# yang-song/score_sde_pytorch

Hardware: AMD Instinct MI355X
Metric: pc_sampler_images_per_sec (higher is better)
Workload: dtype f32 via 3-way bf16 split, fp32 accumulate (the 1x1 / NIN / Linear GEMMs and the attention forward as exact-fp32 products on the BF16 matrix pipe, fp32 softmax; 3x3 convolutions and the attention backward on the fp32-MFMA kernels); 1 GPU; configs/ve/cifar10_ncsnpp_continuous PC sampler (reverse_diffusion+langevin), batch 256/GPU, N=1000, 32x32; 1 step = 1 PC iteration = 2 U-Net evaluations; batch_per_gpu=256, sde_steps=1000, state_finite=True, matrix_mode=bf16x6, parallelism=replicas x1 (no collectives)

## Files before the change

### include/ssde.h

```cpp
#ifndef SSDE_H_
#define SSDE_H_

#include <stddef.h>
#include <stdint.h>

#ifdef __cplusplus
extern "C" {
#endif

#define SSDE_ABI_VERSION 12

enum {
  SSDE_PRO_NONE = 0,
  SSDE_PRO_GN = 1,
  SSDE_PRO_GN_SILU = 2,
  SSDE_PRO_SILU = 3
};

typedef struct ssde_src {
  const float* p0;
  const float* p1;
  int32_t c0, c1;
  int32_t pro_mode;
  int32_t gn_groups;
  const float* gn_mean;
  const float* gn_rstd;
  const float* gn_gamma;
  const float* gn_beta;
  uint32_t drop_thresh;
  float drop_scale;
  const uint32_t* drop_seed;
  uint32_t drop_salt;
  int32_t _pad;
} ssde_src;

typedef struct ssde_conv_args {
  ssde_src main;
  ssde_src aux;
  const float* w_main;
  const float* w_aux;
  int32_t n, h_in, w_in;
  int32_t h_out, w_out, c_out;
  int32_t ksize;
  int32_t stride;
  int32_t pad;
  int32_t tile;
  const float* bias;
  const float* chan_add;
  int32_t chan_add_ld;
  int32_t resid_post;
  const float* resid;
  float out_scale;
  uint32_t flags;
  float* dst;
  float* gn_part;
  float* wino_v;
  const float* gn_in_part0;
  const float* gn_in_part1;
  int32_t gn_in_slices0, gn_in_slices1;
  float gn_in_eps;
  int32_t pad_end;
  float* wino_ws;
  int64_t wino_ws_floats;
} ssde_conv_args;

enum { SSDE_CONVF_V_GIVEN = 1u,
       SSDE_CONVF_BF16X6 = 2u,
       SSDE_CONVF_NO_KSPLIT = 4u,
       SSDE_CONVF_BKC8 = 8u,
       SSDE_CONVF_GEMM_PIPE = 16u,
       SSDE_CONVF_NO_GEMM_PIPE = 32u,
       SSDE_CONVF_X6_BM64 = 64u,
       SSDE_CONVF_X6_PF2 = 128u,
       SSDE_CONVF_NO_SMALL_COUT = 256u,
       SSDE_CONVF_X6_WIDE = 512u,
       SSDE_CONVF_X6_NO_WIDE = 1024u,
       SSDE_CONVF_KSPLIT2 = 2048u,
       SSDE_CONVF_KSPLIT4 = 4096u };
enum { SSDE_TILE_AUTO = 0, SSDE_TILE_256x64 = 1, SSDE_TILE_128x64 = 2, SSDE_TILE_64x64 = 3, SSDE_TILE_256x32 = 4,
       SSDE_TILE_WINOGRAD = 5,
       SSDE_TILE_WINOGRAD4 = 6,
       SSDE_TILE_WINOGRAD4R = 9,
       SSDE_TILE_WINOGRAD4P = 10 };

typedef struct ssde_gn_stats_args {
  const float* p0; const float* p1; int32_t c0, c1;
  int32_t n, hw, groups; float eps;
  float* mean; float* rstd;
  float* scratch;
  int32_t slices; int32_t _pad0;
} ssde_gn_stats_args;

typedef struct ssde_gn_finalize_args {
  const float* part0; const float* part1;
  int32_t c0, c1, slices0, slices1;
  int32_t n, groups; float eps; int32_t _pad0;
  float* mean; float* rstd;
} ssde_gn_finalize_args;

typedef struct ssde_upfirdn_args {
  ssde_src src;
  int32_t n, h_in, w_in, c;
  int32_t h_out, w_out;
  int32_t up, down, pad0, pad1;
  int32_t kh, kw;
  float k[16];
  float* dst;
  int32_t accumulate;
  int32_t _pad0;
  float* dst2;
} ssde_upfirdn_args;

typedef struct ssde_attn_args {
  const float* qkv; float* dst;
  int32_t n, l, c; float scale;
  uint32_t flags;
  int32_t _pad0;
} ssde_attn_args;
enum { SSDE_ATTNF_BF16X6 = 1u };

typedef struct ssde_embed_args {
  const float* cond;
  const float* w;
  float* dst;
  int32_t n, dim, kind, _pad0;
} ssde_embed_args;

typedef struct ssde_to_nhwc_args {
  const float* src; float* dst; int32_t n, c, h, w, c_pad; float a, b;
  int32_t mode;
  const float* v;
} ssde_to_nhwc_args;
typedef struct ssde_to_nchw_args {
  const float* src; float* dst; int32_t n, c, h, w, c_src;
  int32_t mode;
  const float* v;
  float alpha;
  int32_t accumulate;
} ssde_to_nchw_args;

typedef struct ssde_bias_act_args {
  const float* src; const float* bias; float* dst;
  int64_t numel; int32_t channels; int32_t inner;
  int32_t act;
  float alpha, scale;
  int32_t grad;
  const float* ref;
} ssde_bias_act_args;

typedef struct ssde_sumsq_args {
  const float* a; const float* b; float* out_a; float* out_b; int32_t n, per;
} ssde_sumsq_args;
typedef struct ssde_randn_args {
  float* dst; int64_t numel; uint64_t seed; const int32_t* step_ptr; int32_t stream_id; int32_t _pad0;
  const uint64_t* seed_ptr;
} ssde_randn_args;
typedef struct ssde_langevin_args {
  float* x; float* x_mean; const float* grad; const float* noise;
  const float* grad_sumsq; const float* noise_sumsq;
  const float* alpha_tab; const int32_t* step_ptr;
  int32_t n, per; float snr; int32_t _pad0;
} ssde_langevin_args;
typedef struct ssde_predictor_args {
  float* x; float* x_mean; const float* score; const float* noise;
  const float* coef; const int32_t* step_ptr;
  int64_t numel;
} ssde_predictor_args;
typedef struct ssde_sample_update_args {
  const float* x; const float* y; const float* z; const float* a; const float* b; const float* c;
  float* x_mean; float* x_out; int32_t n; int32_t per;
} ssde_sample_update_args;
typedef struct ssde_fill_args {
  float* dst; const float* tab; const int32_t* step_ptr; int32_t n; int32_t _pad0;
} ssde_fill_args;
typedef struct ssde_step_inc_args { int32_t* step_ptr; int32_t delta; int32_t _pad0; } ssde_step_inc_args;
typedef struct ssde_project_args {
  float* x; float* x_mean; const float* data; const float* mask; const float* noise;
  const float* coef; const int32_t* step_ptr;
  int32_t n, c, hw;
  int32_t use_matrix;
  float M[9], invM[9];
} ssde_project_args;



typedef struct ssde_wgrad_args {
  ssde_src src;
  const float* g;
  int32_t g_ld, g_off;
  int32_t n, h_in, w_in, h_out, w_out;
  int32_t c_out;
  int32_t ksize;
  int32_t stride, pad;
  int32_t cin_store;
  int32_t transpose_out;
  int32_t splits;
  float scale;
  uint32_t flags;
  float* dw;
  float* scratch;
  int64_t scratch_floats;
  const float* v_pre;
// ... 277 lines not shown
```

### score_sde_pytorch_amd/_lib.py

```python
import ctypes as C
import os

_HERE = os.path.dirname(os.path.abspath(__file__))
LIB_PATH = os.environ.get("SSDE_LIB_PATH") or os.path.join(_HERE, "libssde_hip.so")
ABI_VERSION = 12

PRO_NONE, PRO_GN, PRO_GN_SILU, PRO_SILU = 0, 1, 2, 3
TILE_AUTO, TILE_256x64, TILE_128x64, TILE_64x64, TILE_256x32, TILE_WINOGRAD, TILE_WINOGRAD4 = 0, 1, 2, 3, 4, 5, 6
TILE_WINOGRAD4R = 9
TILE_WINOGRAD4P = 10
TILES_WINOGRAD4 = (TILE_WINOGRAD4, TILE_WINOGRAD4R, TILE_WINOGRAD4P)
CONVF_V_GIVEN, CONVF_BF16X6, CONVF_NO_KSPLIT, CONVF_BKC8, CONVF_GEMM_PIPE, CONVF_NO_GEMM_PIPE, CONVF_X6_BM64, CONVF_X6_PF2, \
    CONVF_NO_SMALL_COUT, CONVF_X6_WIDE, CONVF_X6_NO_WIDE, CONVF_KSPLIT2, CONVF_KSPLIT4 = 1, 2, 4, 8, 16, 32, 64, 128, 256, 512, 1024, 2048, 4096
WGRADF_DIRECT, WGRADF_F2, WGRADF_F4_FORCE, WGRADF_NO_STREAMK, WGRADF_NO_XCD_ORDER, WGRADF_1X1_CHUNKED, WGRADF_XVEC1 = 1, 2, 4, 8, 16, 32, 64
GNBWDF_THREE_KERNELS, GNBWDF_DEFER_PARAMS = 1, 2
(OP_CONV, OP_GN_STATS, OP_UPFIRDN, OP_ATTN, OP_EMBED, OP_TO_NHWC, OP_TO_NCHW, OP_BIAS_ACT, OP_SUMSQ,
 OP_RANDN, OP_LANGEVIN, OP_PREDICTOR, OP_FILL, OP_STEP_INC, OP_WGRAD, OP_COLSUM, OP_GN_BWD_REDUCE, OP_PROLOGUE_BWD,
 OP_ATTN_BWD, OP_PERTURB, OP_DSM_LOSS, OP_SUMSQ_FLAT, OP_ADAM, OP_MEMSET, OP_AXPY, OP_PACK, OP_PROJECT,
 OP_GN_FINALIZE, OP_PF_DRIFT, OP_HUTCH_DIV, OP_COLSUM_FINISH, OP_GN_BWD_FINISH) = range(1, 33)
FINISH_JOBS = 16
COLSUMF_DEFER = 1
PACK_CONV3, PACK_WINO3, PACK_MATRIX, PACK_VECTOR, PACK_WINO4, PACK_WINO4R, PACK_WINO4P = 1, 2, 3, 4, 5, 6, 7

_fp = C.c_void_p


class Src(C.Structure):
    _fields_ = [("p0", _fp), ("p1", _fp), ("c0", C.c_int32), ("c1", C.c_int32),
                ("pro_mode", C.c_int32), ("gn_groups", C.c_int32),
                ("gn_mean", _fp), ("gn_rstd", _fp), ("gn_gamma", _fp), ("gn_beta", _fp),
                ("drop_thresh", C.c_uint32), ("drop_scale", C.c_float), ("drop_seed", _fp),
                ("drop_salt", C.c_uint32), ("_pad", C.c_int32)]


class ConvArgs(C.Structure):
    _fields_ = [("main", Src), ("aux", Src), ("w_main", _fp), ("w_aux", _fp),
                ("n", C.c_int32), ("h_in", C.c_int32), ("w_in", C.c_int32),
                ("h_out", C.c_int32), ("w_out", C.c_int32), ("c_out", C.c_int32),
                ("ksize", C.c_int32), ("stride", C.c_int32), ("pad", C.c_int32), ("tile", C.c_int32),
                ("bias", _fp), ("chan_add", _fp), ("chan_add_ld", C.c_int32), ("resid_post", C.c_int32),
                ("resid", _fp), ("out_scale", C.c_float), ("flags", C.c_uint32), ("dst", _fp), ("gn_part", _fp), ("wino_v", _fp),
                ("gn_in_part0", _fp), ("gn_in_part1", _fp), ("gn_in_slices0", C.c_int32), ("gn_in_slices1", C.c_int32),
                ("gn_in_eps", C.c_float), ("pad_end", C.c_int32), ("wino_ws", _fp), ("wino_ws_floats", C.c_int64)]


class GnStatsArgs(C.Structure):
    _fields_ = [("p0", _fp), ("p1", _fp), ("c0", C.c_int32), ("c1", C.c_int32),
                ("n", C.c_int32), ("hw", C.c_int32), ("groups", C.c_int32), ("eps", C.c_float),
                ("mean", _fp), ("rstd", _fp), ("scratch", _fp), ("slices", C.c_int32), ("_pad0", C.c_int32)]


class RkCombineArgs(C.Structure):
    _fields_ = [("y", _fp), ("k", _fp), ("n", C.c_int64), ("terms", C.c_int32), ("_pad0", C.c_int32), ("coef", C.c_double * 7),
                ("dst", _fp), ("dst32", _fp), ("n32", C.c_int64)]


class RkErrorArgs(C.Structure):
    _fields_ = [("y", _fp), ("y_new", _fp), ("k", _fp), ("n", C.c_int64), ("coef", C.c_double * 7), ("atol", C.c_double),
                ("rtol", C.c_double), ("partial", _fp), ("partial_len", C.c_int32), ("_pad0", C.c_int32), ("out", _fp)]


class PfDriftArgs(C.Structure):
    _fields_ = [("x", _fp), ("score", _fp), ("dst", _fp), ("numel", C.c_int64), ("a", C.c_float), ("g2", C.c_float), ("dyn", _fp)]


class OdeDyn(C.Structure):
    _fields_ = [("label", C.c_float), ("std", C.c_float), ("a", C.c_float), ("g2", C.c_float), ("dst", _fp)]


class HutchDivArgs(C.Structure):
    _fields_ = [("gx", _fp), ("eps", _fp), ("dst", _fp), ("dst_off", C.c_int64), ("n", C.c_int32), ("per", C.c_int32),
                ("a", C.c_float), ("g2", C.c_float), ("dyn", _fp)]


class GnFinalizeArgs(C.Structure):
    _fields_ = [("part0", _fp), ("part1", _fp), ("c0", C.c_int32), ("c1", C.c_int32), ("slices0", C.c_int32), ("slices1", C.c_int32),
                ("n", C.c_int32), ("groups", C.c_int32), ("eps", C.c_float), ("_pad0", C.c_int32), ("mean", _fp), ("rstd", _fp)]


class UpfirdnArgs(C.Structure):
    _fields_ = [("src", Src), ("n", C.c_int32), ("h_in", C.c_int32), ("w_in", C.c_int32), ("c", C.c_int32),
                ("h_out", C.c_int32), ("w_out", C.c_int32),
                ("up", C.c_int32), ("down", C.c_int32), ("pad0", C.c_int32), ("pad1", C.c_int32),
                ("kh", C.c_int32), ("kw", C.c_int32), ("k", C.c_float * 16), ("dst", _fp),
                ("accumulate", C.c_int32), ("_pad0", C.c_int32), ("dst2", _fp)]


class AttnArgs(C.Structure):
    _fields_ = [("qkv", _fp), ("dst", _fp), ("n", C.c_int32), ("l", C.c_int32), ("c", C.c_int32), ("scale", C.c_float),
                ("flags", C.c_uint32), ("_pad0", C.c_int32)]


class EmbedArgs(C.Structure):
    _fields_ = [("cond", _fp), ("w", _fp), ("dst", _fp), ("n", C.c_int32), ("dim", C.c_int32),
                ("kind", C.c_int32), ("_pad0", C.c_int32)]


class ToNhwcArgs(C.Structure):
    _fields_ = [("src", _fp), ("dst", _fp), ("n", C.c_int32), ("c", C.c_int32), ("h", C.c_int32), ("w", C.c_int32),
                ("c_pad", C.c_int32), ("a", C.c_float), ("b", C.c_float), ("mode", C.c_int32), ("v", _fp)]


class ToNchwArgs(C.Structure):
    _fields_ = [("src", _fp), ("dst", _fp), ("n", C.c_int32), ("c", C.c_int32), ("h", C.c_int32), ("w", C.c_int32),
                ("c_src", C.c_int32), ("mode", C.c_int32), ("v", _fp), ("alpha", C.c_float), ("accumulate", C.c_int32)]


class BiasActArgs(C.Structure):
    _fields_ = [("src", _fp), ("bias", _fp), ("dst", _fp), ("numel", C.c_int64), ("channels", C.c_int32),
                ("inner", C.c_int32), ("act", C.c_int32), ("alpha", C.c_float), ("scale", C.c_float), ("grad", C.c_int32),
                ("ref", _fp)]


class SumsqArgs(C.Structure):
    _fields_ = [("a", _fp), ("b", _fp), ("out_a", _fp), ("out_b", _fp), ("n", C.c_int32), ("per", C.c_int32)]


class RandnArgs(C.Structure):
    _fields_ = [("dst", _fp), ("numel", C.c_int64), ("seed", C.c_uint64), ("step_ptr", _fp),
                ("stream_id", C.c_int32), ("_pad0", C.c_int32), ("seed_ptr", _fp)]


class LangevinArgs(C.Structure):
    _fields_ = [("x", _fp), ("x_mean", _fp), ("grad", _fp), ("noise", _fp), ("grad_sumsq", _fp), ("noise_sumsq", _fp),
                ("alpha_tab", _fp), ("step_ptr", _fp), ("n", C.c_int32), ("per", C.c_int32), ("snr", C.c_float),
                ("_pad0", C.c_int32)]


class PredictorArgs(C.Structure):
    _fields_ = [("x", _fp), ("x_mean", _fp), ("score", _fp), ("noise", _fp), ("coef", _fp), ("step_ptr", _fp),
                ("numel", C.c_int64)]


class SampleUpdateArgs(C.Structure):
    _fields_ = [("x", _fp), ("y", _fp), ("z", _fp), ("a", _fp), ("b", _fp), ("c", _fp), ("x_mean", _fp), ("x_out", _fp),
                ("n", C.c_int32), ("per", C.c_int32)]


class FillArgs(C.Structure):
    _fields_ = [("dst", _fp), ("tab", _fp), ("step_ptr", _fp), ("n", C.c_int32), ("_pad0", C.c_int32)]


class StepIncArgs(C.Structure):
    _fields_ = [("step_ptr", _fp), ("delta", C.c_int32), ("_pad0", C.c_int32)]


class ProjectArgs(C.Structure):
    _fields_ = [("x", _fp), ("x_mean", _fp), ("data", _fp), ("mask", _fp), ("noise", _fp), ("coef", _fp), ("step_ptr", _fp),
                ("n", C.c_int32), ("c", C.c_int32), ("hw", C.c_int32), ("use_matrix", C.c_int32),
                ("M", C.c_float * 9), ("invM", C.c_float * 9)]


class WgradArgs(C.Structure):
    _fields_ = [("src", Src), ("g", _fp), ("g_ld", C.c_int32), ("g_off", C.c_int32),
                ("n", C.c_int32), ("h_in", C.c_int32), ("w_in", C.c_int32), ("h_out", C.c_int32), ("w_out", C.c_int32),
                ("c_out", C.c_int32), ("ksize", C.c_int32), ("stride", C.c_int32), ("pad", C.c_int32),
                ("cin_store", C.c_int32), ("transpose_out", C.c_int32), ("splits", C.c_int32), ("scale", C.c_float),
                ("flags", C.c_uint32), ("dw", _fp), ("scratch", _fp), ("scratch_floats", C.c_int64), ("v_pre", _fp),
                ("pad_end", C.c_int32), ("_pad0", C.c_int32)]


class ColsumArgs(C.Structure):
    _fields_ = [("g", _fp), ("g_ld", C.c_int32), ("g_off", C.c_int32), ("n", C.c_int32), ("hw", C.c_int32),
                ("c", C.c_int32), ("scale", C.c_float), ("per_sample", _fp), ("ps_ld", C.c_int32), ("ps_off", C.c_int32),
                ("total", _fp), ("total2", _fp), ("scratch", _fp), ("flags", C.c_uint32), ("_pad0", C.c_int32)]


class ColsumJob(C.Structure):
    _fields_ = [("part", _fp), ("per_sample", _fp), ("total", _fp), ("total2", _fp), ("n", C.c_int32), ("slices", C.c_int32),
                ("c", C.c_int32), ("ps_ld", C.c_int32), ("ps_off", C.c_int32), ("_pad0", C.c_int32)]


class ColsumFinishArgs(C.Structure):
# ... 47 lines not shown
    _fields_ = [("dst", _fp), ("bytes", C.c_int64), ("value", C.c_int32), ("_pad0", C.c_int32)]


class AxpyArgs(C.Structure):
    _fields_ = [("x", _fp), ("gate", _fp), ("dst", _fp), ("numel", C.c_int64), ("alpha", C.c_float), ("acc", C.c_int32)]


class PackDesc(C.Structure):
    _fields_ = [("src", _fp), ("src2", _fp), ("dst", _fp), ("kind", C.c_int32), ("cout", C.c_int32), ("cin", C.c_int32),
                ("cout_l", C.c_int32), ("cin_l", C.c_int32), ("flags", C.c_int32), ("r_off", C.c_int32), ("c_off", C.c_int32),
                ("n", C.c_int64)]


class PackArgs(C.Structure):
    _fields_ = [("table", _fp), ("count", C.c_int32), ("kind", C.c_int32), ("max_n", C.c_int64)]


class _OpUnion(C.Union):
    _fields_ = [("conv", ConvArgs), ("gn", GnStatsArgs), ("fir", UpfirdnArgs), ("attn", AttnArgs),
                ("embed", EmbedArgs), ("to_nhwc", ToNhwcArgs), ("to_nchw", ToNchwArgs), ("bias_act", BiasActArgs),
                ("sumsq", SumsqArgs), ("randn", RandnArgs), ("langevin", LangevinArgs), ("predictor", PredictorArgs),
                ("fill", FillArgs), ("step_inc", StepIncArgs),
                ("wgrad", WgradArgs), ("colsum", ColsumArgs), ("gn_bwd", GnBwdReduceArgs), ("pro_bwd", PrologueBwdArgs),
                ("attn_bwd", AttnBwdArgs), ("perturb", PerturbArgs), ("dsm_loss", DsmLossArgs),
                ("sumsq_flat", SumsqFlatArgs), ("adam", AdamArgs), ("memset", MemsetArgs), ("axpy", AxpyArgs),
                ("pack", PackArgs), ("project", ProjectArgs), ("gn_fin", GnFinalizeArgs),
                ("pf_drift", PfDriftArgs), ("hutch_div", HutchDivArgs), ("colsum_fin", ColsumFinishArgs), ("gn_bwd_fin", GnBwdFinishArgs)]


class Op(C.Structure):
    _fields_ = [("kind", C.c_int32), ("flops_class", C.c_int32), ("u", _OpUnion)]


_UNION_FIELD = {OP_CONV: "conv", OP_GN_STATS: "gn", OP_UPFIRDN: "fir", OP_ATTN: "attn", OP_EMBED: "embed",
                OP_TO_NHWC: "to_nhwc", OP_TO_NCHW: "to_nchw", OP_BIAS_ACT: "bias_act", OP_SUMSQ: "sumsq",
                OP_RANDN: "randn", OP_LANGEVIN: "langevin", OP_PREDICTOR: "predictor", OP_FILL: "fill",
                OP_STEP_INC: "step_inc", OP_WGRAD: "wgrad", OP_COLSUM: "colsum", OP_GN_BWD_REDUCE: "gn_bwd",
                OP_PROLOGUE_BWD: "pro_bwd", OP_ATTN_BWD: "attn_bwd", OP_PERTURB: "perturb", OP_DSM_LOSS: "dsm_loss",
                OP_SUMSQ_FLAT: "sumsq_flat", OP_ADAM: "adam", OP_MEMSET: "memset", OP_AXPY: "axpy", OP_PACK: "pack", OP_PROJECT: "project",
                OP_GN_FINALIZE: "gn_fin", OP_PF_DRIFT: "pf_drift", OP_HUTCH_DIV: "hutch_div", OP_COLSUM_FINISH: "colsum_fin",
                OP_GN_BWD_FINISH: "gn_bwd_fin"}

EXPORTS = ["ssde_conv2d", "ssde_groupnorm_stats", "ssde_upfirdn2d", "ssde_attention", "ssde_embed", "ssde_to_nhwc",
           "ssde_to_nchw", "ssde_fused_bias_act", "ssde_sumsq", "ssde_randn", "ssde_langevin_update",
           "ssde_predictor_update", "ssde_fill_from_table", "ssde_step_inc", "ssde_program_run",
           "ssde_program_run_timed", "ssde_graph_capture", "ssde_graph_launch", "ssde_graph_destroy",
           "ssde_abi_version", "ssde_sizeof_op", "ssde_last_error", "ssde_conv_lds_bytes",
           "ssde_conv_wgrad", "ssde_colsum", "ssde_gn_bwd_reduce", "ssde_prologue_bwd", "ssde_attention_bwd",
           "ssde_perturb", "ssde_dsm_loss", "ssde_sumsq_flat", "ssde_adam_clip_ema", "ssde_memset", "ssde_axpy",
           "ssde_wgrad_scratch_floats", "ssde_wgrad_wants_winograd4", "ssde_pack_weights", "ssde_project_update", "ssde_gn_finalize", "ssde_conv_gn_slices", "ssde_conv_ws_floats", "ssde_rk_combine", "ssde_rk_error_norm", "ssde_pf_drift", "ssde_hutch_div", "ssde_sample_update", "ssde_mfma_probe", "ssde_colsum_finish", "ssde_gn_bwd_finish", "ssde_gn_bwd_scratch_rows",
           "ssde_plan_load", "ssde_plan_load_file", "ssde_plan_destroy", "ssde_plan_info", "ssde_plan_param",
           "ssde_plan_refresh_weights", "ssde_unet_forward", "ssde_pc_reset", "ssde_pc_run", "ssde_pc_state",
           "ssde_train_step", "ssde_train_forward", "ssde_unet_backward", "ssde_plan_copy_io"]

_lib = None


def conv_route_flags(env=None):
    e = os.environ if env is None else env
    f = 0
    if e.get("SSDE_MATRIX", "").startswith("b"):
        f |= CONVF_BF16X6
    if e.get("SSDE_CONV_KSPLIT", "1") == "0":
        f |= CONVF_NO_KSPLIT
    if e.get("SSDE_CONV_BKC64", "") == "8":
        f |= CONVF_BKC8
    if e.get("SSDE_GEMM_PIPE", "") == "0":
        f |= CONVF_NO_GEMM_PIPE
    if e.get("SSDE_GEMM_PIPE", "") == "2":
        f |= CONVF_GEMM_PIPE
    if e.get("SSDE_X6_BM", "") == "64":
        f |= CONVF_X6_BM64
    if e.get("SSDE_X6_PF", "") == "2":
        f |= CONVF_X6_PF2
    if e.get("SSDE_CONV_SMALL", "1") == "0":
        f |= CONVF_NO_SMALL_COUT
    if e.get("SSDE_X6_WIDE", "") == "1":
        f |= CONVF_X6_WIDE
    if e.get("SSDE_X6_WIDE", "") == "0":
        f |= CONVF_X6_NO_WIDE
    return f


ATTNF_BF16X6 = 1


def attn_route_flags(env=None):
    e = os.environ if env is None else env
    return ATTNF_BF16X6 if e.get("SSDE_MATRIX", "").startswith("b") and e.get("SSDE_ATTN_X6", "1") != "0" else 0


def wgrad_route_flags(env=None):
    e = os.environ if env is None else env
    f = {"0": WGRADF_DIRECT, "2": WGRADF_F2, "44": WGRADF_F4_FORCE}.get(e.get("SSDE_WGRAD_WINOGRAD", ""), 0)
    if e.get("SSDE_WGRAD4_STREAMK", "1") == "0":
        f |= WGRADF_NO_STREAMK
    if e.get("SSDE_WGRAD4_XCD", "1") == "0":
        f |= WGRADF_NO_XCD_ORDER
    if e.get("SSDE_WGRAD_1X1_PIPELINED", "1") == "0":
        f |= WGRADF_1X1_CHUNKED
    if e.get("SSDE_WGRAD4_XVEC", "2") == "1":
        f |= WGRADF_XVEC1
    return f


def gn_bwd_route_flags(env=None):
    e = os.environ if env is None else env
    return GNBWDF_THREE_KERNELS if e.get("SSDE_GN_BWD_FUSED", "1") == "0" else 0


class SsdeError(RuntimeError):
    pass


def bind(lib):
    for name in EXPORTS:
        if not hasattr(lib, name):
            raise SsdeError("libssde_hip.so does not export %s" % name)
    lib.ssde_last_error.restype = C.c_char_p
    lib.ssde_program_run.argtypes = [C.POINTER(Op), C.c_int32, C.c_void_p]
    lib.ssde_program_run_timed.argtypes = [C.POINTER(Op), C.c_int32, C.c_void_p, C.POINTER(C.c_float)]
    lib.ssde_graph_capture.argtypes = [C.POINTER(Op), C.c_int32, C.c_void_p, C.POINTER(C.c_void_p)]
    lib.ssde_graph_launch.argtypes = [C.c_void_p, C.c_void_p]
    lib.ssde_graph_destroy.argtypes = [C.c_void_p]
    for name, typ in [("ssde_conv2d", ConvArgs), ("ssde_groupnorm_stats", GnStatsArgs), ("ssde_upfirdn2d", UpfirdnArgs),
                      ("ssde_attention", AttnArgs), ("ssde_embed", EmbedArgs), ("ssde_to_nhwc", ToNhwcArgs),
                      ("ssde_to_nchw", ToNchwArgs), ("ssde_fused_bias_act", BiasActArgs), ("ssde_sumsq", SumsqArgs),
                      ("ssde_randn", RandnArgs), ("ssde_langevin_update", LangevinArgs),
                      ("ssde_predictor_update", PredictorArgs), ("ssde_fill_from_table", FillArgs),
                      ("ssde_step_inc", StepIncArgs), ("ssde_conv_wgrad", WgradArgs), ("ssde_colsum", ColsumArgs),
                      ("ssde_gn_bwd_reduce", GnBwdReduceArgs), ("ssde_prologue_bwd", PrologueBwdArgs),
                      ("ssde_attention_bwd", AttnBwdArgs), ("ssde_perturb", PerturbArgs), ("ssde_dsm_loss", DsmLossArgs),
                      ("ssde_sumsq_flat", SumsqFlatArgs), ("ssde_adam_clip_ema", AdamArgs), ("ssde_memset", MemsetArgs),
                      ("ssde_axpy", AxpyArgs), ("ssde_pack_weights", PackArgs), ("ssde_project_update", ProjectArgs),
                      ("ssde_gn_finalize", GnFinalizeArgs), ("ssde_rk_combine", RkCombineArgs), ("ssde_hutch_div", HutchDivArgs), ("ssde_sample_update", SampleUpdateArgs),
                      ("ssde_rk_error_norm", RkErrorArgs), ("ssde_pf_drift", PfDriftArgs),
                      ("ssde_colsum_finish", ColsumFinishArgs), ("ssde_gn_bwd_finish", GnBwdFinishArgs)]:
        getattr(lib, name).argtypes = [C.POINTER(typ), C.c_void_p]
    lib.ssde_conv_lds_bytes.argtypes = [C.POINTER(ConvArgs)]
    lib.ssde_conv_gn_slices.argtypes = [C.POINTER(ConvArgs)]
    lib.ssde_conv_ws_floats.argtypes = [C.POINTER(ConvArgs)]
    lib.ssde_conv_ws_floats.restype = C.c_int64
    lib.ssde_wgrad_scratch_floats.argtypes = [C.POINTER(WgradArgs)]
    lib.ssde_wgrad_scratch_floats.restype = C.c_int64
    lib.ssde_wgrad_wants_winograd4.argtypes = [C.POINTER(WgradArgs)]
    lib.ssde_gn_bwd_scratch_rows.argtypes = [C.POINTER(GnBwdReduceArgs)]
    if lib.ssde_abi_version() != ABI_VERSION:
        raise SsdeError("ABI mismatch: library %d, binding %d" % (lib.ssde_abi_version(), ABI_VERSION))
    if lib.ssde_sizeof_op() != C.sizeof(Op):
        raise SsdeError("struct layout mismatch: sizeof(ssde_op) library %d, ctypes %d" % (lib.ssde_sizeof_op(), C.sizeof(Op)))
    return lib


def load():
    global _lib
    if _lib is not None:
        return _lib
    if not os.path.exists(LIB_PATH):
        raise SsdeError(
            "libssde_hip.so not found at %s -- build it with `python -c 'import __graft_entry__ as g; g.build()'` "
            "(score_sde_pytorch_amd has no CPU/eager fallback)" % LIB_PATH)
    lib = bind(C.CDLL(LIB_PATH))
    _lib = lib
    return lib


def check(rc, what=""):
    if rc != 0:
        msg = load().ssde_last_error()
        raise SsdeError("%s failed (%d): %s" % (what or "libssde_hip call", rc, msg.decode() if msg else "?"))


# ... 28 lines not shown
```

### score_sde_pytorch_amd/backward.py

```python
import ctypes as C
import math

import numpy as np
import torch

from . import _lib as L
from . import engine as E
from .engine import _src

FC_WGRAD, FC_BWD = 6, 7


def trainable_params(model):
    frozen = {id(p) for m in model.modules() if getattr(m, "kind", "") == "fourier" for p in m.parameters(recurse=False)}
    return [p for p in model.parameters() if id(p) not in frozen]


class FlatParams:

    def __init__(self, model, device):
        params = trainable_params(model)
        groups = model.flat_param_groups() if hasattr(model, "flat_param_groups") else []
        grouped = [p for g in groups for p in g]
        seen = {id(p) for p in grouped}
# ... 1 lines not shown
        self.model_order = params
        self.index, off = {}, 0
        for p in self.params:
            self.index[id(p)] = (off, p.numel())
            off += (p.numel() + 3) // 4 * 4
        self.numel = off
        self.data = torch.zeros(off, dtype=torch.float32, device=device)
        self.grad = torch.zeros(off, dtype=torch.float32, device=device)
        with torch.no_grad():
            for p in self.params:
                o, n = self.index[id(p)]
                self.data[o:o + n].copy_(p.detach().reshape(-1).to(device, torch.float32))
                p.data = self.data[o:o + n].view(p.shape)
                p._ssde_flat = self
        self.device = device
        self.generation = 0

    def touch(self):
        self.generation += 1

    def owns(self, model):
        ps = trainable_params(model)
        if len(ps) != len(self.params):
            return False
        base = self.data.data_ptr()
        for p in ps:
            e = self.index.get(id(p))
            if e is None or p.data_ptr() != base + e[0] * 4:
                return False
        return True

    def owns_params(self, params):
        base = self.data.data_ptr()
        for p in params:
            e = self.index.get(id(p))
            if e is None or p.data_ptr() != base + e[0] * 4:
                return False
        return True

    def grad_view(self, p):
        o, n = self.index[id(p)]
        return self.grad[o:o + n].view(p.shape)

    def contiguous(self, params):
        for a, b in zip(params[:-1], params[1:]):
            oa, na = self.index[id(a)]
            if self.index[id(b)][0] != oa + na:
                return False
        return True

    def grad_run(self, params):
        o = self.index[id(params[0])][0]
        n = sum(self.index[id(p)][1] for p in params)
        runs = self.__dict__.setdefault("runs", {})
        runs[o] = max(runs.get(o, 0), n)
        return self.grad[o:o + n]

    def write_extent(self, off):
        n = self.__dict__.get("runs", {}).get(off, 0)
        if getattr(self, "_starts", None) is None:
            self._starts = sorted((o, ln) for o, ln in self.index.values())
        import bisect
        i = bisect.bisect_right(self._starts, (off, float("inf"))) - 1
        if i >= 0:
            o, ln = self._starts[i]
            if off < o + ln:
                n = max(n, o + ln - off)
        return max(n, 1)

    def attach_grads(self):
        for p in self.params:
            p.grad = self.grad_view(p)


def flat_params_of(model, device):
    fp = getattr(model, "_flat_params", None)
    if fp is None or fp.device != device or not fp.owns(model):
        fp = FlatParams(model, device)
        model._flat_params = fp
    return fp


class TrainEngine(E.UNetEngine):

    def __init__(self, model, batch, height, width, device, vp_score=False, input_grad=False, dropout=True,
                 param_grads=True):
        self.param_grads = param_grads
        self.flat = flat_params_of(model, device)
        super().__init__(model, batch, height, width, device, vp_score=vp_score, train=bool(dropout), input_grad=input_grad,
                         finalize=False)
        self.n_fwd = len(self.b.specs)
        self.gout = self.b.buf(batch, self.channels, height, width, name="gout", persistent=True)
        self.gx = self.b.buf(batch, self.channels, height, width, name="gx", persistent=True) if input_grad else None
        self._G = {}
        import os
        self.defer_finish = os.environ.get("SSDE_DEFER_FINISH", "1") != "0"
        self._jobs = {L.OP_COLSUM_FINISH: [], L.OP_GN_BWD_FINISH: []}
        self._pending_per = set()
        self._lower_backward()
        self.program = self.b.finalize()
        self.n_fwd = self.program.spec_start[self.n_fwd]
        self.n_bwd = self.program.n - self.n_fwd

    def _needs(self, buf):
        if buf is None:
            return False
        if isinstance(buf, tuple):
            buf = buf[0]
        return id(buf) not in self._nograd

    def _gentry(self, buf):
        e = self._G.get(id(buf))
        if e is None:
            e = self._G[id(buf)] = [self.b.buf(*buf.shape, name="g_" + buf.name), False]
        return e

    def _param_of(self, packed):
        return self.weights.meta[id(packed)]["parts"][0]["param"]

    def _lower_backward(self):
        b = self.b
        self._nograd = {id(self.x_in), id(self.cond), id(self._emb)}
        if self.sig is not self.cond:
            self._nograd.add(id(self.sig))
        if self.std is not None:
            self._nograd.add(id(self.std))
        if not self.input_grad:
            self._nograd.add(id(self._x0))
        fwd = list(b.specs[: self.n_fwd])
        if self.param_grads:
            b.add(L.OP_MEMSET, dict(dst=self.flat.grad, bytes=self.flat.numel * 4, value=0), FC_BWD)
        handlers = {L.OP_CONV: self._bwd_conv, L.OP_UPFIRDN: self._bwd_fir, L.OP_ATTN: self._bwd_attn,
                    L.OP_TO_NCHW: self._bwd_to_nchw, L.OP_TO_NHWC: self._bwd_to_nhwc}
        for kind, f, _, _ in reversed(fwd):
            h = handlers.get(kind)
            if h is not None:
                h(f)
        for kind in list(self._jobs):
            self._flush_finish(kind)

    def _flush_finish(self, kind):
        jobs = self._jobs[kind]
        if jobs:
            self.b.add(kind, dict(count=len(jobs), job=list(jobs)), FC_BWD)
            del jobs[:]
        if kind == L.OP_COLSUM_FINISH:
            self._pending_per.clear()

    def _defer(self, kind, job):
        self._jobs[kind].append(job)
        if len(self._jobs[kind]) == L.FINISH_JOBS:
            self._flush_finish(kind)

    def _colsum(self, fields):
        if not self.defer_finish:
            self.b.add(L.OP_COLSUM, fields, FC_BWD)
            return
        self.b.add(L.OP_COLSUM, dict(fields, per_sample=None, total=None, total2=None, flags=L.COLSUMF_DEFER), FC_BWD)
        if fields["per_sample"] is not None:
            self._pending_per.add(id(fields["per_sample"]))
        self._defer(L.OP_COLSUM_FINISH, dict(part=fields["scratch"], per_sample=fields["per_sample"], total=fields["total"],
                                             total2=fields["total2"], n=fields["n"], slices=max(1, min(32, fields["hw"] // 64)),
                                             c=fields["c"], ps_ld=fields["ps_ld"], ps_off=fields["ps_off"]))

    def _bwd_to_nchw(self, f):
        e = self._gentry(f["src"])
# ... 317 lines not shown
```

### score_sde_pytorch_amd/csrc/attention.hip

```cpp
#include "ssde_common.h"
#include <type_traits>

typedef float f32x16 __attribute__((ext_vector_type(16)));

namespace {

constexpr int kQB = 64;
constexpr int kLMax = 256;
constexpr int kLDC = 36;
constexpr int kLDP = 260;
constexpr int kTileFloats = kQB * kLDP;
constexpr int kStageFloats = (kQB + kLMax) * kLDC;
constexpr int kFwdVch = 8;
constexpr int kAttnLdsFloats = kQB * kLDP + kFwdVch * kLDP;
constexpr int kBwdLdsFloats = kTileFloats + kStageFloats + 3 * kLMax;

__device__ __forceinline__ void zero_acc(f32x16 (&acc)[2][2]) {
#pragma unroll
  for (int a = 0; a < 2; ++a)
#pragma unroll
    for (int b = 0; b < 2; ++b)
#pragma unroll
      for (int r = 0; r < 16; ++r) acc[a][b][r] = 0.f;
}

__device__ __forceinline__ void gemm_nt(const float* __restrict__ A, int a_valid, size_t lda,
                                        const float* __restrict__ B, int b_valid, size_t ldb, int C, int Lk,
                                        float* Qs, float* Ks, f32x16 (&acc)[2][2]) {
  const int tid = threadIdx.x, wave = tid >> 6, lane = tid & 63;
  const int li = lane & 31, lh = lane >> 5;
  const int kb = wave * 64;
  zero_acc(acc);
  const int f = tid & 7, r0 = tid >> 3;
  float4 ra[2], rb[8];
  auto load_chunk = [&](int c0) {
#pragma unroll
    for (int it = 0; it < 2; ++it) {
      const int row = r0 + it * 32;
      const float4 v = *reinterpret_cast<const float4*>(A + (size_t)max(min(row, a_valid - 1), 0) * lda + c0 + f * 4);
      ra[it] = row < a_valid ? v : make_float4(0.f, 0.f, 0.f, 0.f);
    }
#pragma unroll
    for (int it = 0; it < 8; ++it) {
      const int row = r0 + it * 32;
      const float4 v = *reinterpret_cast<const float4*>(B + (size_t)max(min(row, b_valid - 1), 0) * ldb + c0 + f * 4);
      rb[it] = row < b_valid ? v : make_float4(0.f, 0.f, 0.f, 0.f);
    }
  };
  load_chunk(0);
  for (int c0 = 0; c0 < C; c0 += 32) {
    __syncthreads();
#pragma unroll
    for (int it = 0; it < 2; ++it) *reinterpret_cast<float4*>(Qs + (r0 + it * 32) * kLDC + f * 4) = ra[it];
#pragma unroll
    for (int it = 0; it < 8; ++it)
      if (r0 + it * 32 < Lk) *reinterpret_cast<float4*>(Ks + (r0 + it * 32) * kLDC + f * 4) = rb[it];
    __syncthreads();
    if (c0 + 32 < C) load_chunk(c0 + 32);
    if (kb < Lk) {
#pragma unroll
      for (int kk = 0; kk < 4; ++kk) {
        float4 af[2], bf[2];
#pragma unroll
        for (int a = 0; a < 2; ++a) af[a] = *reinterpret_cast<const float4*>(Qs + (a * 32 + li) * kLDC + kk * 8 + lh * 4);
#pragma unroll
        for (int b = 0; b < 2; ++b) bf[b] = *reinterpret_cast<const float4*>(Ks + (kb + b * 32 + li) * kLDC + kk * 8 + lh * 4);
#pragma unroll
        for (int a = 0; a < 2; ++a)
#pragma unroll
          for (int b = 0; b < 2; ++b) {
            acc[a][b] = __builtin_amdgcn_mfma_f32_32x32x2f32(af[a].x, bf[b].x, acc[a][b], 0, 0, 0);
            acc[a][b] = __builtin_amdgcn_mfma_f32_32x32x2f32(af[a].y, bf[b].y, acc[a][b], 0, 0, 0);
            acc[a][b] = __builtin_amdgcn_mfma_f32_32x32x2f32(af[a].z, bf[b].z, acc[a][b], 0, 0, 0);
            acc[a][b] = __builtin_amdgcn_mfma_f32_32x32x2f32(af[a].w, bf[b].w, acc[a][b], 0, 0, 0);
          }
      }
    }
  }
}

template <int VCH = 32>
__device__ __forceinline__ void gemm_pv(const float* Ps, int Lp, const float* __restrict__ Bm, int b_valid, size_t ldb, int C,
                                        float* Vs, float* __restrict__ out, size_t ldo, int out_valid, float out_scale) {
  const int tid = threadIdx.x, wave = tid >> 6, lane = tid & 63;
// ... 65 lines not shown
          if (col >= C) continue;
#pragma unroll
          for (int r = 0; r < 16; ++r) {
            const int row = a * 32 + (r & 3) + 8 * (r >> 2) + 4 * lh;
            if (row < out_valid) out[(size_t)row * ldo + col] = acc[a][b][r] * out_scale;
          }
        }
    }
  }
}

__device__ __forceinline__ void acc_to_tile(const f32x16 (&acc)[2][2], float* Ps, int Lk, float mul) {
  const int wave = threadIdx.x >> 6, lane = threadIdx.x & 63;
  const int li = lane & 31, lh = lane >> 5, kb = wave * 64;
  if (kb < Lk) {
#pragma unroll
    for (int a = 0; a < 2; ++a)
#pragma unroll
      for (int b = 0; b < 2; ++b)
#pragma unroll
        for (int r = 0; r < 16; ++r) {
          const int row = a * 32 + (r & 3) + 8 * (r >> 2) + 4 * lh;
          Ps[row * kLDP + kb + b * 32 + li] = acc[a][b][r] * mul;
        }
  }
}

__device__ __forceinline__ void softmax_rows(float* Ps, int L, float* m_out, float* l_out) {
  const int tid = threadIdx.x;
  const int row = tid >> 2, sub = tid & 3;
  float* prow = Ps + row * kLDP;
  float m = -INFINITY;
  for (int j = sub; j < L; j += 4) m = fmaxf(m, prow[j]);
  m = fmaxf(m, __shfl_xor(m, 1, 64));
  m = fmaxf(m, __shfl_xor(m, 2, 64));
  float sum = 0.f;
  for (int j = sub; j < L; j += 4) { const float e = __expf(prow[j] - m); prow[j] = e; sum += e; }
  sum += __shfl_xor(sum, 1, 64);
  sum += __shfl_xor(sum, 2, 64);
  const float inv = 1.0f / sum;
  for (int j = sub; j < L; j += 4) prow[j] *= inv;
  const int Lp = (L + 31) & ~31;
  for (int j = L + sub; j < Lp; j += 4) prow[j] = 0.f;
  *m_out = m; *l_out = sum;
}

__global__ __launch_bounds__(256) void attn_kernel(const float* __restrict__ qkv, float* __restrict__ dst,
                                                   int N, int L, int C, float scale) {
  SSDE_LDS(smem);
  float* Qs = smem;
  float* Ks = smem + kQB * kLDC;
  float* Ps = smem;
  float* Vs = smem + kQB * kLDP;
  const int n = blockIdx.y, q0 = blockIdx.x * kQB;
  const int C3 = 3 * C;
  const float* base = qkv + (size_t)n * L * C3;
  const int Lk = (L + 63) & ~63;
  const int Lp = (L + 31) & ~31;

  f32x16 acc[2][2];
  gemm_nt(base + (size_t)q0 * C3, L - q0, C3, base + C, L, C3, C, Lk, Qs, Ks, acc);
  __syncthreads();
  acc_to_tile(acc, Ps, Lk, scale);
  __syncthreads();
  float m, l;
  softmax_rows(Ps, L, &m, &l);
  gemm_pv<kFwdVch>(Ps, Lp, base + 2 * C, L, C3, C, Vs, dst + ((size_t)n * L + q0) * C, C, L - q0, 1.0f);
}

namespace x6 {
constexpr int kT = 512, kRows = 64, kL = 256;
constexpr int kKStage = 3 * kL * 32;
constexpr int kPPlane = kL * kRows * 2;
constexpr int kMain = 3 * kPPlane;
constexpr int kLds = kMain + 2 * kKStage;
static_assert(kRows * kLDP * 4 <= kMain, "score tile");

__device__ __forceinline__ void split_hi(float x, uint32_t& a, uint32_t& b, uint32_t& c) {
  a = __builtin_bit_cast(uint32_t, x);
  const float r = x - __builtin_bit_cast(float, a & 0xffff0000u);
  b = __builtin_bit_cast(uint32_t, r);
  c = __builtin_bit_cast(uint32_t, r - __builtin_bit_cast(float, b & 0xffff0000u));
}
}

template <int kNst>
__global__ __launch_bounds__(x6::kT) void attn_x6_kernel(const float* __restrict__ qkv, float* __restrict__ dst, int N, float scale) {
  using namespace x6;
  constexpr int C = 16 * kNst;
  SSDE_LDS(smem);
  char* lds = reinterpret_cast<char*>(smem);
  char* stage0 = lds + kMain;
  char* stage1 = stage0 + kKStage;
  const int tid = threadIdx.x, lane = tid & 63;
  const int wave = __builtin_amdgcn_readfirstlane(tid >> 6);
  const int li = lane & 31, lh = lane >> 5;
  const int xcd = blockIdx.x & 7, k_in = blockIdx.x >> 3;
  const int n = (k_in >> 2) * 8 + xcd, q0 = (k_in & 3) * kRows;
  if (n >= N) return;
  const int C3 = 3 * C;
  const float* base = qkv + (size_t)n * kL * C3;
  const int qplane = C * kRows * 2;
  constexpr int nst = kNst;

  const bool consumer = wave < 4;
  f32x16 acc[2][2];
  auto zero = [&]() {
#pragma unroll
    for (int a = 0; a < 2; ++a)
#pragma unroll
      for (int b = 0; b < 2; ++b)
#pragma unroll
        for (int r = 0; r < 16; ++r) acc[a][b][r] = 0.f;
  };
  struct Frags { ssde_u32x4 A[2][3], B[2][3]; };
  auto read_frags = [&](Frags& f, const char* ap, int a_pitch, const char* bp, int b_pitch) __attribute__((always_inline)) {
#pragma unroll
    for (int q = 0; q < 3; ++q) {
#pragma unroll
      for (int a = 0; a < 2; ++a) f.A[a][q] = *reinterpret_cast<const ssde_u32x4*>(ap + q * a_pitch + (a * 32 + li) * 32 + lh * 16);
#pragma unroll
      for (int b = 0; b < 2; ++b) f.B[b][q] = *reinterpret_cast<const ssde_u32x4*>(bp + q * b_pitch + (wave * 64 + b * 32 + li) * 32 + lh * 16);
    }
  };
  auto mfmas = [&](auto Terms, const Frags& f) __attribute__((always_inline)) {
    constexpr int kTerms = decltype(Terms)::value;
    constexpr int TI[8] = {1, 2, 0, 2, 1, 0, 1, 0}, TJ[8] = {2, 1, 2, 0, 1, 1, 0, 0};
#pragma unroll
    for (int t = 8 - kTerms; t < 8; ++t)
#pragma unroll
      for (int a = 0; a < 2; ++a)
#pragma unroll
        for (int b = 0; b < 2; ++b)
          acc[a][b] = __builtin_amdgcn_mfma_f32_32x32x16_bf16(__builtin_bit_cast(ssde_bf16x8, f.A[a][TI[t]]),
                                                              __builtin_bit_cast(ssde_bf16x8, f.B[b][TJ[t]]), acc[a][b], 0, 0, 0);
  };
  using Six = std::integral_constant<int, 6>;
  using Eight = std::integral_constant<int, 8>;

  const int ptid = tid & 255;
  const float* kbase = base + C;
  const float* vbase = base + 2 * C;
  const int krow = ptid >> 2, kf = ptid & 3;
  const uint32_t koff = (uint32_t)((krow * C3 + kf * 4) * 4), kstep = (uint32_t)(64 * C3 * 4);
  const int tp = ptid & 7, fq0 = ptid >> 3;
  const bool v_on0 = fq0 * 4 < C, v_on1 = (fq0 + 32) * 4 < C;
  const uint32_t voff = (uint32_t)((2 * tp * C3 + (v_on0 ? fq0 * 4 : 0)) * 4), vtok = (uint32_t)(C3 * 4), vquad = v_on1 ? 512u : 0u;
  const int vpitch = C * 32;
  auto request = [&](int u, ssde_f32x4 (&Rs)[4]) __attribute__((always_inline)) {
    const bool is_k = u < nst;
    const float* sb = is_k ? kbase + u * 16 : vbase + (size_t)(u - nst) * 16 * C3;
    const uint32_t o0 = is_k ? koff : voff;
    const uint32_t o1 = o0 + (is_k ? kstep : vtok);
    const uint32_t o2 = is_k ? o0 + 2 * kstep : o0 + vquad;
    const uint32_t o3 = is_k ? o0 + 3 * kstep : o2 + vtok;
    SSDE_GLOAD16_I_SAFE(Rs[0], o0, sb, 0);
    SSDE_GLOAD16_I_SAFE(Rs[1], o1, sb, 0);
    SSDE_GLOAD16_I_SAFE(Rs[2], o2, sb, 0);
    SSDE_GLOAD16_I_SAFE(Rs[3], o3, sb, 0);
  };
#ifdef SSDE_EMULATED
#define SSDE_X6_WAIT(n, Rs) ((void)0)
#else
#define SSDE_X6_WAIT(n, Rs) asm volatile("s_waitcnt vmcnt(%4)" : "+v"((Rs)[0]), "+v"((Rs)[1]), "+v"((Rs)[2]), "+v"((Rs)[3]) : "n"(n) : "memory")
#endif
  auto park_k = [&](const ssde_f32x4 (&Rs)[4], char* buf) __attribute__((always_inline)) {
#pragma unroll
    for (int i = 0; i < 4; ++i) {
      uint2 p0, p1, p2;
      ssde_split3(make_float4(Rs[i].x, Rs[i].y, Rs[i].z, Rs[i].w), p0, p1, p2);
      char* d = buf + (krow + 64 * i) * 32 + kf * 8;
      *reinterpret_cast<uint2*>(d) = p0;
      *reinterpret_cast<uint2*>(d + kL * 32) = p1;
      *reinterpret_cast<uint2*>(d + 2 * kL * 32) = p2;
    }
  };
  const int rot = (fq0 >> 1) & 3;
  const bool rot1 = (rot & 1) != 0, rot2 = (rot & 2) != 0;
  auto park_v = [&](const ssde_f32x4 (&Rs)[4], char* buf) __attribute__((always_inline)) {
#pragma unroll
    for (int h = 0; h < 2; ++h) {
      const float f0[4] = {Rs[2 * h].x, Rs[2 * h].y, Rs[2 * h].z, Rs[2 * h].w};
      const float f1[4] = {Rs[2 * h + 1].x, Rs[2 * h + 1].y, Rs[2 * h + 1].z, Rs[2 * h + 1].w};
      uint32_t w[3][4], y[3][4];
#pragma unroll
      for (int i = 0; i < 4; ++i) {
        uint32_t a0, b0, c0, a1, b1, c1;
        split_hi(f0[i], a0, b0, c0);
        split_hi(f1[i], a1, b1, c1);
        w[0][i] = ssde_pack_hi16(a0, a1); w[1][i] = ssde_pack_hi16(b0, b1); w[2][i] = ssde_pack_hi16(c0, c1);
      }
#pragma unroll
      for (int q = 0; q < 3; ++q) {
        uint32_t x[4];
#pragma unroll
        for (int i = 0; i < 4; ++i) x[i] = rot1 ? w[q][(i + 1) & 3] : w[q][i];
#pragma unroll
        for (int i = 0; i < 4; ++i) y[q][i] = rot2 ? x[(i + 2) & 3] : x[i];
      }
      if (h == 0 ? v_on0 : v_on1) {
#pragma unroll
        for (int j = 0; j < 4; ++j) {
          char* d = buf + ((fq0 + 32 * h) * 4 + ((j + rot) & 3)) * 32 + tp * 4;
#pragma unroll
          for (int q = 0; q < 3; ++q) *reinterpret_cast<uint32_t*>(d + q * vpitch) = y[q][j];
        }
      }
    }
  };

  ssde_f32x4 R[4][4];
  zero();
  if (!consumer) { request(0, R[0]); request(1, R[1]); request(2, R[2]); request(3, R[3]); }
  {
    const int cq4 = C >> 2, total = kRows * cq4;
    for (int item0 = tid; item0 < total; item0 += 8 * kT) {
      float4 qv[8];
#pragma unroll
      for (int u = 0; u < 8; ++u) {
        const int item = min(item0 + u * kT, total - 1);
        const int row = item / cq4, cq = item - row * cq4;
        qv[u] = *reinterpret_cast<const float4*>(base + (size_t)(q0 + row) * C3 + cq * 4);
      }
#pragma unroll
      for (int u = 0; u < 8; ++u) {
        const int item = item0 + u * kT;
        if (item < total) {
          const int row = item / cq4, cq = item - row * cq4;
          uint2 p0, p1, p2;
          ssde_split3(qv[u], p0, p1, p2);
          char* d = lds + (cq >> 2) * (kRows * 32) + row * 32 + (cq & 3) * 8;
          *reinterpret_cast<uint2*>(d) = p0;
          *reinterpret_cast<uint2*>(d + qplane) = p1;
          *reinterpret_cast<uint2*>(d + 2 * qplane) = p2;
        }
      }
    }
  }
  if (consumer) {
    SSDE_LDS_BARRIER();
    for (int u = 0; u < nst; ++u) {
      Frags f;
      read_frags(f, lds + u * (kRows * 32), qplane, (u & 1) ? stage1 : stage0, kL * 32);
      mfmas(Eight{}, f);
      SSDE_LDS_BARRIER();
    }
  } else {
    SSDE_X6_WAIT(12, R[0]);
    park_k(R[0], stage0);
    SSDE_LDS_BARRIER();
#pragma unroll
    for (int u = 0; u < nst; ++u) {
      const int j = u & 3;
      request(u + 4, R[j]);
      SSDE_X6_WAIT(12, R[(j + 1) & 3]);
      if (u + 1 < nst) park_k(R[(j + 1) & 3], (j & 1) ? stage0 : stage1);
      SSDE_LDS_BARRIER();
    }
    SSDE_X6_WAIT(8, R[1]); SSDE_X6_WAIT(4, R[2]); SSDE_X6_WAIT(0, R[3]);
  }

  {
    float* tile = smem;
    if (consumer) {
#pragma unroll
      for (int a = 0; a < 2; ++a)
#pragma unroll
        for (int b = 0; b < 2; ++b)
#pragma unroll
          for (int r = 0; r < 16; ++r) {
            const int row = a * 32 + (r & 3) + 8 * (r >> 2) + 4 * lh;
            tile[row * kLDP + wave * 64 + b * 32 + li] = acc[a][b][r] * scale;
          }
    }
    SSDE_LDS_BARRIER();
    const int row = tid >> 3, sub = tid & 7;
    float x[32];
#pragma unroll
    for (int i = 0; i < 8; ++i) {
      const float4 v = *reinterpret_cast<const float4*>(tile + row * kLDP + sub * 32 + i * 4);
      x[4 * i] = v.x; x[4 * i + 1] = v.y; x[4 * i + 2] = v.z; x[4 * i + 3] = v.w;
    }
    SSDE_LDS_BARRIER();
    float m = x[0];
#pragma unroll
    for (int i = 1; i < 32; ++i) m = fmaxf(m, x[i]);
    m = fmaxf(m, __shfl_xor(m, 1, 64));
    m = fmaxf(m, __shfl_xor(m, 2, 64));
    m = fmaxf(m, __shfl_xor(m, 4, 64));
    float sum = 0.f;
#pragma unroll
    for (int i = 0; i < 32; ++i) { x[i] = __expf(x[i] - m); sum += x[i]; }
    sum += __shfl_xor(sum, 1, 64);
    sum += __shfl_xor(sum, 2, 64);
    sum += __shfl_xor(sum, 4, 64);
    const float inv = 1.0f / sum;
#pragma unroll
    for (int u = 0; u < 4; ++u) {
      uint2 a0, a1, a2, b0, b1, b2;
      ssde_split3(make_float4(x[8 * u] * inv, x[8 * u + 1] * inv, x[8 * u + 2] * inv, x[8 * u + 3] * inv), a0, a1, a2);
      ssde_split3(make_float4(x[8 * u + 4] * inv, x[8 * u + 5] * inv, x[8 * u + 6] * inv, x[8 * u + 7] * inv), b0, b1, b2);
      char* d = lds + (2 * sub + (u >> 1)) * (kRows * 32) + row * 32 + (u & 1) * 16;
      *reinterpret_cast<uint4*>(d) = make_uint4(a0.x, a0.y, b0.x, b0.y);
      *reinterpret_cast<uint4*>(d + kPPlane) = make_uint4(a1.x, a1.y, b1.x, b1.y);
      *reinterpret_cast<uint4*>(d + 2 * kPPlane) = make_uint4(a2.x, a2.y, b2.x, b2.y);
    }
  }

  if (consumer) {
    const bool w_on = wave * 64 < C;
    zero();
    SSDE_LDS_BARRIER();
    for (int v = 0; v < 16; ++v) {
      if (w_on) {
        Frags f;
        read_frags(f, lds + v * (kRows * 32), kPPlane, (v & 1) ? stage1 : stage0, vpitch);
        mfmas(Six{}, f);
      }
      SSDE_LDS_BARRIER();
    }
    if (w_on) {
#pragma unroll
      for (int b = 0; b < 2; ++b) {
        float* out = dst + ((size_t)n * kL + q0) * C + wave * 64 + b * 32 + li;
#pragma unroll
        for (int a = 0; a < 2; ++a)
#pragma unroll
          for (int r = 0; r < 16; ++r) {
            const int row = a * 32 + (r & 3) + 8 * (r >> 2) + 4 * lh;
            out[(size_t)row * C] = acc[a][b][r];
          }
      }
    }
  } else {
    park_v(R[0], stage0);
    SSDE_LDS_BARRIER();
#pragma unroll
    for (int v = 0; v < 16; ++v) {
      const int j = v & 3;
      if (v + 4 < 16) request(nst + v + 4, R[j]);
      if (v + 1 < 16) {
        if (v + 1 >= 4) {
          if (v + 4 < 16) SSDE_X6_WAIT(12, R[(j + 1) & 3]);
          else if (v + 3 < 16) SSDE_X6_WAIT(8, R[(j + 1) & 3]);
          else if (v + 2 < 16) SSDE_X6_WAIT(4, R[(j + 1) & 3]);
          else SSDE_X6_WAIT(0, R[(j + 1) & 3]);
        }
        park_v(R[(j + 1) & 3], (j & 1) ? stage0 : stage1);
      }
      SSDE_LDS_BARRIER();
    }
  }
#undef SSDE_X6_WAIT
}

__global__ __launch_bounds__(256) void attn_bwd_q_kernel(const float* __restrict__ qkv, const float* __restrict__ o,
                                                         const float* __restrict__ d_o, float* __restrict__ dqkv,
                                                         float* __restrict__ stats, int N, int L, int C, float scale) {
  SSDE_LDS(smem);
  float* Ps = smem;
  float* Qs = smem + kTileFloats;
  float* Ks = Qs + kQB * kLDC;
  float* Vs = Qs;
  float* Ds = smem + kTileFloats + kStageFloats;
  const int n = blockIdx.y, q0 = blockIdx.x * kQB, tid = threadIdx.x;
  const int C3 = 3 * C;
  const float* base = qkv + (size_t)n * L * C3;
  const int Lk = (L + 63) & ~63, Lp = (L + 31) & ~31;
  const int valid = L - q0;

  f32x16 acc[2][2];
  gemm_nt(base + (size_t)q0 * C3, valid, C3, base + C, L, C3, C, Lk, Qs, Ks, acc);
  __syncthreads();
  acc_to_tile(acc, Ps, Lk, scale);
  __syncthreads();
  float m, l;
  softmax_rows(Ps, L, &m, &l);
  {
    const int row = tid >> 2, sub = tid & 3;
    float d = 0.f;
    if (row < valid) {
      const float* po = o + ((size_t)n * L + q0 + row) * C;
      const float* pd = d_o + ((size_t)n * L + q0 + row) * C;
      for (int c = sub * 4; c < C; c += 16) {
        const float4 a = *reinterpret_cast<const float4*>(po + c);
        const float4 b = *reinterpret_cast<const float4*>(pd + c);
        d += (a.x * b.x + a.y * b.y) + (a.z * b.z + a.w * b.w);
      }
    }
    d += __shfl_xor(d, 1, 64);
    d += __shfl_xor(d, 2, 64);
    if (sub == 0) {
      Ds[row] = d;
      if (row < valid) {
        float* st = stats + ((size_t)n * L + q0 + row) * 4;
        st[0] = m; st[1] = l; st[2] = d; st[3] = 0.f;
      }
    }
  }
  gemm_nt(d_o + ((size_t)n * L + q0) * C, valid, C, base + 2 * C, L, C3, C, Lk, Qs, Ks, acc);
  __syncthreads();
  {
    const int wave = tid >> 6, lane = tid & 63, li = lane & 31, lh = lane >> 5, kb = wave * 64;
    if (kb < Lk) {
#pragma unroll
      for (int a = 0; a < 2; ++a)
#pragma unroll
        for (int b = 0; b < 2; ++b)
#pragma unroll
          for (int r = 0; r < 16; ++r) {
            const int row = a * 32 + (r & 3) + 8 * (r >> 2) + 4 * lh;
            const int col = kb + b * 32 + li;
            if (col < Lp) Ps[row * kLDP + col] *= (acc[a][b][r] - Ds[row]);
          }
    }
  }
  gemm_pv(Ps, Lp, base + C, L, C3, C, Vs, dqkv + ((size_t)n * L + q0) * C3, C3, valid, scale);
}

__global__ __launch_bounds__(256) void attn_bwd_kv_kernel(const float* __restrict__ qkv, const float* __restrict__ d_o,
                                                          float* __restrict__ dqkv, const float* __restrict__ stats,
                                                          int N, int L, int C, float scale) {
  SSDE_LDS(smem);
  float* Ps = smem;
  float* Qs = smem + kTileFloats;
  float* Ks = Qs + kQB * kLDC;
  float* Vs = Qs;
  float* St = smem + kTileFloats + kStageFloats;
  const int n = blockIdx.y, k0 = blockIdx.x * kQB, tid = threadIdx.x;
  const int C3 = 3 * C;
  const float* base = qkv + (size_t)n * L * C3;
  const int Lk = (L + 63) & ~63, Lp = (L + 31) & ~31;
  const int valid = L - k0;
  for (int j = tid; j < kLMax; j += 256) {
    float m = 0.f, l = 1.f, d = 0.f;
    if (j < L) { const float* st = stats + ((size_t)n * L + j) * 4; m = st[0]; l = st[1]; d = st[2]; }
    St[j] = m; St[kLMax + j] = l; St[2 * kLMax + j] = d;
  }
  const int wave = tid >> 6, lane = tid & 63, li = lane & 31, lh = lane >> 5, kb = wave * 64;

  f32x16 acc[2][2];
  gemm_nt(base + (size_t)k0 * C3 + C, valid, C3, base, L, C3, C, Lk, Qs, Ks, acc);
  __syncthreads();
  if (kb < Lk) {
#pragma unroll
    for (int a = 0; a < 2; ++a)
#pragma unroll
      for (int b = 0; b < 2; ++b)
#pragma unroll
        for (int r = 0; r < 16; ++r) {
          const int row = a * 32 + (r & 3) + 8 * (r >> 2) + 4 * lh;
          const int col = kb + b * 32 + li;
          float pv = 0.f;
          if (row < valid && col < L) pv = __expf(acc[a][b][r] * scale - St[col]) / St[kLMax + col];
          Ps[row * kLDP + col] = pv;
        }
  }
  __syncthreads();
  gemm_pv(Ps, Lp, d_o + (size_t)n * L * C, L, C, C, Vs, dqkv + ((size_t)n * L + k0) * C3 + 2 * C, C3, valid, 1.0f);
  gemm_nt(base + (size_t)k0 * C3 + 2 * C, valid, C3, d_o + (size_t)n * L * C, L, C, C, Lk, Qs, Ks, acc);
  __syncthreads();
  if (kb < Lk) {
#pragma unroll
    for (int a = 0; a < 2; ++a)
#pragma unroll
      for (int b = 0; b < 2; ++b)
#pragma unroll
        for (int r = 0; r < 16; ++r) {
          const int row = a * 32 + (r & 3) + 8 * (r >> 2) + 4 * lh;
          const int col = kb + b * 32 + li;
          if (col < Lp) Ps[row * kLDP + col] *= (acc[a][b][r] - St[2 * kLMax + col]);
        }
  }
  gemm_pv(Ps, Lp, base, L, C3, C, Vs, dqkv + ((size_t)n * L + k0) * C3 + C, C3, valid, scale);
}

template <typename K>
int set_lds_once(K kfn, int bytes, std::atomic<bool>* done) {
  if (!*done) {
    SSDE_HIP_CHECK(hipFuncSetAttribute(reinterpret_cast<const void*>(kfn), hipFuncAttributeMaxDynamicSharedMemorySize, bytes));
    *done = true;
  }
  return SSDE_OK;
}

}

extern "C" int ssde_attention(const ssde_attn_args* a, void* stream) {
  SSDE_REQUIRE(a && a->qkv && a->dst, "attention: null args");
  SSDE_REQUIRE(a->n > 0 && a->l > 0 && a->l <= kLMax, "attention: token count %d outside 1..%d", a->l, kLMax);
  SSDE_REQUIRE(a->c > 0 && a->c % 32 == 0, "attention: channels must be a multiple of 32 (got %d)", a->c);
  if ((a->flags & SSDE_ATTNF_BF16X6) && a->l == x6::kL && a->c <= 256 && a->c % 64 == 0) {
    static std::atomic<bool> x6_set[4];
    const dim3 grid(ssde_cdiv(a->n, 8) * 8 * 4);
    hipStream_t st = static_cast<hipStream_t>(stream);
#define SSDE_ATTN_X6_GO(NST, SLOT)                                                                       \
    do {                                                                                                 \
      if (int rc = set_lds_once(attn_x6_kernel<NST>, x6::kLds, &x6_set[SLOT])) return rc;                \
      hipLaunchKernelGGL(attn_x6_kernel<NST>, grid, dim3(x6::kT), x6::kLds, st, a->qkv, a->dst, a->n, a->scale); \
    } while (0)
    switch (a->c) {
      case 64: SSDE_ATTN_X6_GO(4, 0); break;
      case 128: SSDE_ATTN_X6_GO(8, 1); break;
      case 192: SSDE_ATTN_X6_GO(12, 2); break;
      default: SSDE_ATTN_X6_GO(16, 3); break;
    }
#undef SSDE_ATTN_X6_GO
    SSDE_LAUNCH_CHECK();
    return SSDE_OK;
  }
  const int lds = kAttnLdsFloats * 4;
  static std::atomic<bool> attr_set{false};
  if (int rc = set_lds_once(attn_kernel, lds, &attr_set)) return rc;
  hipLaunchKernelGGL(attn_kernel, dim3(ssde_cdiv(a->l, kQB), a->n), dim3(256), lds, static_cast<hipStream_t>(stream),
                     a->qkv, a->dst, a->n, a->l, a->c, a->scale);
  SSDE_LAUNCH_CHECK();
  return SSDE_OK;
}

extern "C" int ssde_attention_bwd(const ssde_attn_bwd_args* a, void* stream) {
  SSDE_REQUIRE(a && a->qkv && a->o && a->d_o && a->dqkv && a->stats, "attention_bwd: null args");
  SSDE_REQUIRE(a->n > 0 && a->l > 0 && a->l <= kLMax, "attention_bwd: token count %d outside 1..%d", a->l, kLMax);
  SSDE_REQUIRE(a->c > 0 && a->c % 32 == 0, "attention_bwd: channels must be a multiple of 32 (got %d)", a->c);
  const int lds = kBwdLdsFloats * 4;
  static std::atomic<bool> set_q{false}, set_kv{false};
  if (int rc = set_lds_once(attn_bwd_q_kernel, lds, &set_q)) return rc;
  if (int rc = set_lds_once(attn_bwd_kv_kernel, lds, &set_kv)) return rc;
  hipStream_t st = static_cast<hipStream_t>(stream);
  const dim3 grid(ssde_cdiv(a->l, kQB), a->n);
  hipLaunchKernelGGL(attn_bwd_q_kernel, grid, dim3(256), lds, st, a->qkv, a->o, a->d_o, a->dqkv, a->stats, a->n, a->l, a->c, a->scale);
  SSDE_LAUNCH_CHECK();
  hipLaunchKernelGGL(attn_bwd_kv_kernel, grid, dim3(256), lds, st, a->qkv, a->d_o, a->dqkv, a->stats, a->n, a->l, a->c, a->scale);
  SSDE_LAUNCH_CHECK();
  return SSDE_OK;
}
```

### score_sde_pytorch_amd/csrc/conv1x1.hip

```cpp
#include "ssde_common.h"

typedef float f32x16 __attribute__((ext_vector_type(16)));

#ifdef SSDE_GEMM_TRACE
__device__ unsigned long long* g_gemm_trace;
extern "C" int ssde_debug_gemm_trace(void* buf) {
  return hipMemcpyToSymbol(HIP_SYMBOL(g_gemm_trace), &buf, sizeof(buf)) == hipSuccess ? 0 : -5;
}
#define SSDE_GT(slot)                                                                  \
  do {                                                                                 \
    if (gt_on) g_gemm_trace[(slot)] = __builtin_amdgcn_s_memtime();                    \
  } while (0)
__device__ unsigned long long* g_gemm_wg_trace;
extern "C" int ssde_debug_gemm_wg_trace(void* buf) {
  return hipMemcpyToSymbol(HIP_SYMBOL(g_gemm_wg_trace), &buf, sizeof(buf)) == hipSuccess ? 0 : -5;
}
#define SSDE_GW(slot)                                                                                          \
  do {                                                                                                         \
    if (threadIdx.x == 0 && g_gemm_wg_trace != nullptr) {                                                      \
      g_gemm_wg_trace[(size_t)blockIdx.x * 4 + (slot)] = __builtin_amdgcn_s_memtime();                         \
      if ((slot) == 0) g_gemm_wg_trace[(size_t)blockIdx.x * 4 + 3] = __builtin_amdgcn_s_getreg((4 << 0) | (0 << 6) | (31 << 11)) | ((unsigned long long)__builtin_amdgcn_s_getreg((20 << 0) | (0 << 6) | (3 << 11)) << 32); \
    }                                                                                                          \
  } while (0)
#else
#define SSDE_GT(slot) do { } while (0)
#define SSDE_GW(slot) do { } while (0)
#endif

#ifndef SSDE_GEMM_BATCH
#define SSDE_GEMM_BATCH 1
#endif
#ifndef SSDE_GEMM_OCC
#define SSDE_GEMM_OCC 4
#endif

namespace {

constexpr int kThreads = 256;
constexpr int BM = 128, BN = 128, BK = 16, LDK = 18;
constexpr int kStage = (BM + BN) * LDK;

struct GemmParams {
  ssde_src src;
  const float* wpk;
  int M, HW, K, Cout, CoutPad, m_tiles, n_tiles;
  const float* bias; const float* chan_add; int chan_add_ld;
  const float* resid; int resid_post;
  float scale;
  float* dst;
  float* gn_part;
  int lHW, gn_entries;
};

template <bool kGn>
__global__ __launch_bounds__(kThreads, SSDE_GEMM_OCC) void gemm1x1_kernel(const GemmParams p) {
  SSDE_LDS(smem);
  const int tid = threadIdx.x, wave = tid >> 6, lane = tid & 63;
  const int li = lane & 31, lh = lane >> 5;
  const int xcd = blockIdx.x & 7, lin = blockIdx.x >> 3;
  const int nt = lin % p.n_tiles, mt = (lin / p.n_tiles) * 8 + xcd;
#ifdef SSDE_GEMM_TRACE
  const bool gt_on = tid == 0 && blockIdx.x == 0 && g_gemm_trace != nullptr;
#endif
  SSDE_GT(0);
  if (mt >= p.m_tiles) return;
  const int m0 = mt * BM, n0 = nt * BN;
  const int wm0 = (wave >> 1) * 64, wn0 = (wave & 1) * 64;
  const ssde_src& s = p.src;
  SsdePro pro = ssde_pro_decode(s);
  pro.gn = kGn;
  const int Ctot = s.c0 + s.c1;
  const int cpg = kGn ? Ctot / s.gn_groups : 1;
  const int nst = (p.K + BK - 1) / BK;
  const int ncin8 = (p.K + 7) >> 3;

  constexpr int NI = 2, RS = 64;
  const int f = tid & 3, r0 = tid >> 2;
  int arow[NI], aimg[NI];
  bool aok[NI];
#pragma unroll
  for (int i = 0; i < NI; ++i) {
    const int m = m0 + r0 + i * RS;
    aok[i] = m < p.M;
    arow[i] = aok[i] ? m : 0;
    aimg[i] = arow[i] / p.HW;
  }
  bool bok[NI];
#pragma unroll
  for (int i = 0; i < NI; ++i) bok[i] = (n0 + r0 + i * RS) < p.CoutPad;
  const float* bptr = p.wpk + ((size_t)n0 + r0) * 8 + (f & 1) * 4;

  float4 av[NI], bv[NI];
  float mu[NI], rs[NI];
  float4 gam = make_float4(1.f, 1.f, 1.f, 1.f), bet = make_float4(0.f, 0.f, 0.f, 0.f);
  bool k_ok = false;
  int c_cur = 0;

  auto load_stage = [&](int st) {
    const int c_base = st * BK;
    const bool second = c_base >= s.c0;
    const float* base = second ? s.p1 : s.p0;
    const int C = second ? s.c1 : s.c0;
    const int cthr = (second ? c_base - s.c0 : c_base) + f * 4;
    c_cur = c_base + f * 4;
    k_ok = c_cur < p.K;
    const float* ap = base + (k_ok ? cthr : 0);
#pragma unroll
    for (int i = 0; i < NI; ++i) av[i] = *reinterpret_cast<const float4*>(ap + (size_t)arow[i] * C);
    const int cin8 = min(st * 2 + (f >> 1), ncin8 - 1);
    const float* bp = bptr + (size_t)cin8 * p.CoutPad * 8;
#pragma unroll
    for (int i = 0; i < NI; ++i) bv[i] = *reinterpret_cast<const float4*>(bp + (bok[i] ? i * RS * 8 : 0));
    if (kGn) {
      const int cg = k_ok ? c_cur : 0;
      gam = *reinterpret_cast<const float4*>(s.gn_gamma + cg);
      bet = *reinterpret_cast<const float4*>(s.gn_beta + cg);
#pragma unroll
      for (int i = 0; i < NI; ++i) {
        const int gi = aimg[i] * s.gn_groups + cg / cpg;
        mu[i] = s.gn_mean[gi];
        rs[i] = s.gn_rstd[gi];
      }
    }
  };
  auto store_stage = [&](int st, float* buf) {
    const int cin8 = st * 2 + (f >> 1);
#pragma unroll
    for (int i = 0; i < NI; ++i) {
      float4 v = make_float4(0.f, 0.f, 0.f, 0.f);
      if (aok[i] && k_ok)
        v = ssde_pro_apply(av[i], mu[i], rs[i], gam, bet, (uint32_t)arow[i] * (uint32_t)Ctot + (uint32_t)c_cur, pro);
      float* d = buf + (r0 + i * RS) * LDK + f * 4;
      *reinterpret_cast<float2*>(d) = make_float2(v.x, v.y);
      *reinterpret_cast<float2*>(d + 2) = make_float2(v.z, v.w);
// ... 21 lines not shown

  SSDE_GT(1);
  load_stage(0);
  store_stage(0, smem);
  __syncthreads();
  SSDE_GT(2);
  for (int st = 0; st < nst; ++st) {
    const float* cur = smem + (st & 1) * kStage;
    const bool has_next = st + 1 < nst;
    if (has_next) load_stage(st + 1);
    float2 af[2][2], bf[2][2];
#pragma unroll
    for (int a = 0; a < 2; ++a) af[0][a] = *reinterpret_cast<const float2*>(cur + aoff[a]);
#pragma unroll
    for (int b = 0; b < 2; ++b) bf[0][b] = *reinterpret_cast<const float2*>(cur + boff[b]);
#pragma unroll
    for (int t = 0; t < BK / 4; ++t) {
      const int c = t & 1;
      if (t + 1 < BK / 4) {
#pragma unroll
        for (int a = 0; a < 2; ++a) af[c ^ 1][a] = *reinterpret_cast<const float2*>(cur + aoff[a] + (t + 1) * 4);
#pragma unroll
        for (int b = 0; b < 2; ++b) bf[c ^ 1][b] = *reinterpret_cast<const float2*>(cur + boff[b] + (t + 1) * 4);
      }
#pragma unroll
      for (int a = 0; a < 2; ++a)
#pragma unroll
        for (int b = 0; b < 2; ++b) acc[a][b] = __builtin_amdgcn_mfma_f32_32x32x2f32(af[c][a].x, bf[c][b].x, acc[a][b], 0, 0, 0);
#pragma unroll
      for (int a = 0; a < 2; ++a)
#pragma unroll
        for (int b = 0; b < 2; ++b) acc[a][b] = __builtin_amdgcn_mfma_f32_32x32x2f32(af[c][a].y, bf[c][b].y, acc[a][b], 0, 0, 0);
      if (t + 1 < BK / 4) __builtin_amdgcn_sched_group_barrier(0x100, 4, 0);
      __builtin_amdgcn_sched_group_barrier(0x008, 8, 0);
    }
    if (st < 8) SSDE_GT(4 + st * 4);
    if (has_next) store_stage(st + 1, smem + ((st + 1) & 1) * kStage);
    if (st < 8) SSDE_GT(5 + st * 4);
    __syncthreads();
    if (st < 8) SSDE_GT(6 + st * 4);
  }
  SSDE_GT(40);

  constexpr int LDT = BN + 4;
  SsdeEpi e{p.bias, p.chan_add, p.chan_add_ld, p.resid, p.resid_post, p.scale, p.dst, p.Cout, p.gn_part};
#pragma unroll
  for (int half = 0; half < 2; ++half) {
    if ((wave >> 1) == half) {
#pragma unroll
      for (int b = 0; b < 2; ++b)
#pragma unroll
        for (int a = 0; a < 2; ++a)
#pragma unroll
          for (int r = 0; r < 16; ++r) {
            const int m = a * 32 + (r & 3) + 8 * (r >> 2) + 4 * lh;
            smem[m * LDT + wn0 + b * 32 + li] = acc[a][b][r];
          }
    }
    __syncthreads();
    ssde_store_tile<64, BN, kThreads, SSDE_GEMM_BATCH>(smem, LDT, n0, e, [&](int row, size_t& pix, int& img) {
      const int m = m0 + half * 64 + row;
      if (m >= p.M) return false;
      pix = (size_t)m;
      img = m / p.HW;
      return true;
    }, p.gn_part ? (p.HW >= 64 ? (m0 >> 6) + half : (m0 + half * 64) / p.HW) : -1, p.HW >= 64 ? 30 : p.lHW, p.gn_entries);
    SSDE_GT(41 + half * 2);
    __syncthreads();
    SSDE_GT(42 + half * 2);
  }
}

#ifndef SSDE_X6_PF2_OCC_LOSS
#define SSDE_X6_PF2_OCC_LOSS 1
#endif
constexpr int XBK = 16;
template <int kBM, int kBN = 128> struct X6 {
  static constexpr int kPlaneA = kBM * XBK * 2, kPlaneB = kBN * XBK * 2;
  static constexpr int kStageBytes = 3 * kPlaneA + 3 * kPlaneB;
  static constexpr int NA = kBM / 64;
  static constexpr int NBW = kBN / 64;
};

template <bool kGn, int kBM, int kPF, int kBN = 128>
__global__ __launch_bounds__(kThreads, kBN == 256 ? 2 : (kBM == 64 ? 4 : 3) - (kPF == 2 ? SSDE_X6_PF2_OCC_LOSS : 0)) void gemm1x1_bf16x6_kernel(const GemmParams p) {
  using X = X6<kBM, kBN>;
  constexpr int NA = X::NA, NB = X::NBW, NBW = X::NBW, RS = 64;
  SSDE_LDS(smem);
  char* lds = reinterpret_cast<char*>(smem);
  const int tid = threadIdx.x, wave = tid >> 6, lane = tid & 63;
  const int li = lane & 31, lh = lane >> 5;
  const int xcd = blockIdx.x & 7, lin = blockIdx.x >> 3;
  const int nt = lin % p.n_tiles, mt = (lin / p.n_tiles) * 8 + xcd;
#ifdef SSDE_GEMM_TRACE
  const bool gt_on = tid == 0 && blockIdx.x == 0 && g_gemm_trace != nullptr;
#endif
  SSDE_GT(0);
  if (mt >= p.m_tiles) return;
  SSDE_GW(0);
  const int m0 = mt * kBM, n0 = nt * kBN;
  const int wm0 = (wave >> 1) * (kBM / 2), wn0 = (wave & 1) * (kBN / 2);
  const ssde_src& s = p.src;
  SsdePro pro = ssde_pro_decode(s);
  pro.gn = kGn;
  const int Ctot = s.c0 + s.c1;
  const int cpg = kGn ? Ctot / s.gn_groups : 1;
  const int nst = (p.K + XBK - 1) / XBK;
  const int ncin8 = (p.K + 7) >> 3;

  const int f = tid & 3, r0 = tid >> 2;
  int arow[NA], aimg[NA];
  bool aok[NA];
#pragma unroll
  for (int i = 0; i < NA; ++i) {
    const int m = m0 + r0 + i * RS;
    aok[i] = m < p.M;
    arow[i] = aok[i] ? m : 0;
    aimg[i] = arow[i] / p.HW;
  }
  bool bok[NB];
#pragma unroll
  for (int i = 0; i < NB; ++i) bok[i] = (n0 + r0 + i * RS) < p.CoutPad;
  const float* bptr = p.wpk + ((size_t)n0 + r0) * 8 + (f & 1) * 4;

  struct ARegs { float4 av[NA]; };
  struct StageRegs {
    float4 bv[NB];
    float mu[NA], rs[NA];
    float4 gam, bet;
  };
  auto load_a = [&](int st, ARegs& A) __attribute__((always_inline)) {
    const int c_base = st * XBK;
    const bool second = c_base >= s.c0;
    const float* base = second ? s.p1 : s.p0;
    const int C = second ? s.c1 : s.c0;
    const int cthr = (second ? c_base - s.c0 : c_base) + f * 4;
    const float* ap = base + (c_base + f * 4 < p.K ? cthr : 0);
#pragma unroll
    for (int i = 0; i < NA; ++i) A.av[i] = *reinterpret_cast<const float4*>(ap + (size_t)arow[i] * C);
  };
  auto load_rest = [&](int st, StageRegs& R) __attribute__((always_inline)) {
    const int c_cur = st * XBK + f * 4;
    const int cin8 = min(st * 2 + (f >> 1), ncin8 - 1);
    const float* bp = bptr + (size_t)cin8 * p.CoutPad * 8;
#pragma unroll
    for (int i = 0; i < NB; ++i) R.bv[i] = *reinterpret_cast<const float4*>(bp + (bok[i] ? i * RS * 8 : 0));
    R.gam = make_float4(1.f, 1.f, 1.f, 1.f); R.bet = make_float4(0.f, 0.f, 0.f, 0.f);
#pragma unroll
    for (int i = 0; i < NA; ++i) { R.mu[i] = 0.f; R.rs[i] = 1.f; }
    if (kGn) {
      const int cg = c_cur < p.K ? c_cur : 0;
      R.gam = *reinterpret_cast<const float4*>(s.gn_gamma + cg);
      R.bet = *reinterpret_cast<const float4*>(s.gn_beta + cg);
#pragma unroll
      for (int i = 0; i < NA; ++i) {
        const int gi = aimg[i] * s.gn_groups + cg / cpg;
        R.mu[i] = s.gn_mean[gi];
        R.rs[i] = s.gn_rstd[gi];
      }
    }
  };
  auto store_stage = [&](int st, const ARegs& A, const StageRegs& R, char* buf) __attribute__((always_inline)) {
    const int cin8 = st * 2 + (f >> 1);
    const int c_cur = st * XBK + f * 4;
    const bool k_ok = c_cur < p.K;
    uint2 q0, q1, q2;
#pragma unroll
// ... 43 lines not shown
        for (int b = 0; b < 2; ++b) B[b][q] = *reinterpret_cast<const ssde_u32x4*>(cur + boff + q * X::kPlaneB + (b0 + b) * 32 * (XBK * 2));
#pragma unroll
      for (int t = 0; t < 6; ++t)
#pragma unroll
        for (int a = 0; a < NA; ++a)
#pragma unroll
          for (int b = 0; b < 2; ++b)
            acc[a][b0 + b] = __builtin_amdgcn_mfma_f32_32x32x16_bf16(__builtin_bit_cast(ssde_bf16x8, A[a][TI[t]]),
                                                                     __builtin_bit_cast(ssde_bf16x8, B[b][TJ[t]]), acc[a][b0 + b], 0, 0, 0);
    }
  };

  SSDE_GT(1);
  char* buf0 = lds;
  char* buf1 = lds + X::kStageBytes;
  StageRegs R;
  if constexpr (kPF == 1) {
    ARegs A0;
    load_a(0, A0); load_rest(0, R);
    store_stage(0, A0, R, buf0);
    __syncthreads();
    SSDE_GT(2);
    for (int st = 0; st < nst; ++st) {
      const bool has_next = st + 1 < nst;
      if (has_next) { load_a(st + 1, A0); load_rest(st + 1, R); }
      mfma_stage((st & 1) ? buf1 : buf0);
      if (st < 8) SSDE_GT(4 + st * 4);
      if (has_next) store_stage(st + 1, A0, R, (st & 1) ? buf0 : buf1);
      if (st < 8) SSDE_GT(5 + st * 4);
      __syncthreads();
      if (st < 8) SSDE_GT(6 + st * 4);
    }
  } else {
    ARegs A0, A1;
    const int last = nst - 1;
    load_a(0, A0); load_rest(0, R);
    load_a(min(1, last), A1);
    store_stage(0, A0, R, buf0);
    __syncthreads();
    SSDE_GT(2);
    for (int st = 0; st < nst; st += 2) {
      load_rest(min(st + 1, last), R);
      __builtin_amdgcn_sched_barrier(0);
      load_a(min(st + 2, last), A0);
      __builtin_amdgcn_sched_barrier(0);
      mfma_stage(buf0);
      if (st < 8) SSDE_GT(4 + st * 4);
      if (st + 1 < nst) store_stage(st + 1, A1, R, buf1);
      if (st < 8) SSDE_GT(5 + st * 4);
      __syncthreads();
      if (st < 8) SSDE_GT(6 + st * 4);
      if (st + 1 >= nst) break;
      load_rest(min(st + 2, last), R);
      __builtin_amdgcn_sched_barrier(0);
      load_a(min(st + 3, last), A1);
      __builtin_amdgcn_sched_barrier(0);
      mfma_stage(buf1);
      if (st + 1 < 8) SSDE_GT(4 + (st + 1) * 4);
      if (st + 2 < nst) store_stage(st + 2, A0, R, buf0);
      if (st + 1 < 8) SSDE_GT(5 + (st + 1) * 4);
      __syncthreads();
      if (st + 1 < 8) SSDE_GT(6 + (st + 1) * 4);
    }
  }
  SSDE_GT(40);
  SSDE_GW(1);

  constexpr int LDT = kBN + 4;
  SsdeEpi e{p.bias, p.chan_add, p.chan_add_ld, p.resid, p.resid_post, p.scale, p.dst, p.Cout, p.gn_part};
#pragma unroll
  for (int half = 0; half < kBM / 64; ++half) {
    if (kBM == 64 || (wave >> 1) == half) {
#pragma unroll
      for (int b = 0; b < NBW; ++b)
#pragma unroll
        for (int a = 0; a < NA; ++a)
#pragma unroll
          for (int r = 0; r < 16; ++r) {
            const int m = (kBM == 64 ? wm0 : 0) + a * 32 + (r & 3) + 8 * (r >> 2) + 4 * lh;
            smem[m * LDT + wn0 + b * 32 + li] = acc[a][b][r];
          }
    }
    __syncthreads();
    ssde_store_tile<64, kBN, kThreads, SSDE_GEMM_BATCH>(smem, LDT, n0, e, [&](int row, size_t& pix, int& img) {
      const int m = m0 + half * 64 + row;
      if (m >= p.M) return false;
      pix = (size_t)m;
      img = m / p.HW;
      return true;
    }, p.gn_part ? (p.HW >= 64 ? (m0 >> 6) + half : (m0 + half * 64) / p.HW) : -1, p.HW >= 64 ? 30 : p.lHW, p.gn_entries);
    SSDE_GT(41 + half * 2);
    __syncthreads();
    SSDE_GT(42 + half * 2);
  }
  SSDE_GW(2);
}

constexpr int kSlabLd = 68;
constexpr int kSlabFloats = 8 * kSlabLd;

template <bool kGn, bool kX6>
__global__ __launch_bounds__(kThreads, 2) void gemm1x1_pipe_kernel(const GemmParams p) {
  SSDE_LDS(smem);
  constexpr int kStageB = kX6 ? X6<128>::kStageBytes : kStage * 4;
  constexpr int KB = 16;
  char* lds = reinterpret_cast<char*>(smem);
  const int tid = threadIdx.x, wave = tid >> 6, lane = tid & 63;
  const int li = lane & 31, lh = lane >> 5;
  float* slab = reinterpret_cast<float*>(lds + 2 * kStageB) + wave * kSlabFloats;
  const int wm0 = (wave >> 1) * 64, wn0 = (wave & 1) * 64;
  const ssde_src& s = p.src;
  SsdePro pro = ssde_pro_decode(s);
  pro.gn = kGn;
  const int Ctot = s.c0 + s.c1;
  const int cpg = kGn ? Ctot / s.gn_groups : 1;
  const int nst = (p.K + KB - 1) / KB;
  const int ncin8 = (p.K + 7) >> 3;
  const int f = tid & 3, r0 = tid >> 2;
  constexpr int NI = 2, RS = 64;
  const int d_row = lane >> 4, d_c4 = lane & 15;

  struct Pending {
    int m0, n0, done;
    bool valid;
    float4 bias4;
    float4 rnext[2];
    float st_p, st_s1, st_s2, st_n;
  };
  Pending pd;
  pd.valid = false; pd.done = 8; pd.m0 = pd.n0 = 0;
  pd.bias4 = make_float4(0.f, 0.f, 0.f, 0.f);
  pd.rnext[0] = pd.rnext[1] = make_float4(0.f, 0.f, 0.f, 0.f);
  pd.st_p = pd.st_s1 = pd.st_s2 = pd.st_n = 0.f;

  auto unit_row = [&](int u, int k) {
    int r = wm0 + (u >> 2) * 32 + (u & 3) * 8 + d_row;
    SSDE_OPAQUE_VGPR(r);
    return r + 4 * k;
  };
  auto fetch_resid = [&](int u) __attribute__((always_inline)) {
#pragma unroll
    for (int k = 0; k < 2; ++k) {
      const int m = pd.m0 + unit_row(u, k), j = pd.n0 + wn0 + d_c4 * 4;
      pd.rnext[k] = make_float4(0.f, 0.f, 0.f, 0.f);
      if (p.resid && u < 8 && m < p.M && j < p.Cout) pd.rnext[k] = *reinterpret_cast<const float4*>(p.resid + (size_t)m * p.Cout + j);
    }
  };
  auto drain_unit = [&](auto A_, auto Q_, f32x16 (&acc)[2][2]) __attribute__((always_inline)) {
    constexpr int a = decltype(A_)::value, q = decltype(Q_)::value, u = a * 4 + q;
    const float4 rr[2] = {pd.rnext[0], pd.rnext[1]};
    fetch_resid(u + 1);
    SSDE_WAVE_SYNC();
#pragma unroll
    for (int b = 0; b < 2; ++b)
#pragma unroll
      for (int r = 0; r < 4; ++r) slab[(r + 4 * lh) * kSlabLd + b * 32 + li] = acc[a][b][4 * q + r];
    SSDE_WAVE_SYNC();
    const int j = pd.n0 + wn0 + d_c4 * 4;
    const int img = p.chan_add ? (pd.m0 + unit_row(u, 0) - d_row) / p.HW : 0;
#pragma unroll
    for (int k = 0; k < 2; ++k) {
      const float4 t = *reinterpret_cast<const float4*>(slab + (d_row + 4 * k) * kSlabLd + d_c4 * 4);
      const int m = pd.m0 + unit_row(u, k);
      if (m < p.M && j < p.Cout) {
        float4 ca = make_float4(0.f, 0.f, 0.f, 0.f);
        if (p.chan_add) ca = *reinterpret_cast<const float4*>(p.chan_add + (size_t)img * p.chan_add_ld + j);
// ... 172 lines not shown
#pragma unroll
          for (int a = 0; a < 2; ++a)
#pragma unroll
            for (int b = 0; b < 2; ++b) acc[a][b] = __builtin_amdgcn_mfma_f32_32x32x2f32(af[c][a].y, bf[c][b].y, acc[a][b], 0, 0, 0);
        }
      }
    };
#pragma unroll
    for (int a = 0; a < 2; ++a)
#pragma unroll
      for (int b = 0; b < 2; ++b)
#pragma unroll
        for (int r = 0; r < 16; ++r) acc[a][b][r] = 0.f;
    char* buf0 = lds;
    char* buf1 = lds + kStageB;
    load_stage(0);
    store_stage(0, buf0);
    __syncthreads();
    for (int st = 0; st < nst; ++st) {
      const bool has_next = st + 1 < nst;
      if (has_next) load_stage(st + 1);
      mfma_stage((st & 1) ? buf1 : buf0);
      if (pd.valid) {
        const int target = ((st + 1) * 8 + nst - 1) / nst;
        while (pd.done < target && pd.done < 8) drain_next(old);
      }
      if (has_next) store_stage(st + 1, (st & 1) ? buf0 : buf1);
      __syncthreads();
    }
    if (pd.valid) finish_tile(old);
    pd.valid = true; pd.done = 0; pd.m0 = m0; pd.n0 = n0;
    pd.st_p = pd.st_s1 = pd.st_s2 = pd.st_n = 0.f;
    pd.bias4 = make_float4(0.f, 0.f, 0.f, 0.f);
    const int j = n0 + wn0 + d_c4 * 4;
    if (p.bias && j < p.Cout) pd.bias4 = *reinterpret_cast<const float4*>(p.bias + j);
    fetch_resid(0);
  };

  f32x16 acc[2][2], old[2][2];
  const int total_vb = ((p.m_tiles + 7) / 8) * 8 * p.n_tiles;
  for (int vb = blockIdx.x; vb < total_vb; vb += gridDim.x) {
    if (((vb >> 3) / p.n_tiles) * 8 + (vb & 7) >= p.m_tiles) continue;
    run_tile(vb, acc, old);
#pragma unroll
    for (int a = 0; a < 2; ++a)
#pragma unroll
      for (int b = 0; b < 2; ++b) old[a][b] = acc[a][b];
  }
  if (pd.valid) finish_tile(old);
}

}

bool ssde_conv1x1_wants(const ssde_conv_args* a) {
  if (a->ksize != 0 || a->aux.p0 == nullptr || a->tile != SSDE_TILE_AUTO) return false;
  const long long M = (long long)a->n * a->h_out * a->w_out;
  return a->c_out >= 96 && M >= 128 && M < (1ll << 31);
}

int ssde_conv1x1_launch(const ssde_conv_args* a, void* stream, int* lds_out) {
  const ssde_src& s = a->aux;
  SSDE_REQUIRE(s.c0 % 4 == 0 && s.c1 % 4 == 0, "conv1x1: channels must be multiples of 4 (got %d,%d)", s.c0, s.c1);
  SSDE_REQUIRE(s.c1 == 0 || (s.p1 != nullptr && s.c0 % 32 == 0), "conv1x1: concat boundary must be a multiple of 32");
  const bool gn = s.pro_mode == SSDE_PRO_GN || s.pro_mode == SSDE_PRO_GN_SILU;
  if (gn) {
    SSDE_REQUIRE(s.gn_groups > 0 && (s.c0 + s.c1) % s.gn_groups == 0 && ((s.c0 + s.c1) / s.gn_groups) % 4 == 0,
                 "conv1x1: GroupNorm needs channels-per-group %% 4 == 0");
    SSDE_REQUIRE(s.gn_mean && s.gn_rstd && s.gn_gamma && s.gn_beta, "conv1x1: GroupNorm pointers missing");
  }
  SSDE_REQUIRE(a->w_aux && a->dst, "conv1x1: null weights / destination");
  GemmParams p;
  p.src = s; p.wpk = a->w_aux;
  p.M = a->n * a->h_out * a->w_out; p.HW = a->h_out * a->w_out; p.K = s.c0 + s.c1;
  p.Cout = a->c_out; p.CoutPad = ssde_cdiv(a->c_out, 64) * 64;
  p.m_tiles = ssde_cdiv(p.M, BM); p.n_tiles = ssde_cdiv(a->c_out, BN);
  p.bias = a->bias; p.chan_add = a->chan_add; p.chan_add_ld = a->chan_add_ld;
  p.resid = a->resid; p.resid_post = a->resid_post; p.scale = a->out_scale; p.dst = a->dst;
  p.gn_part = a->gn_part;
  const bool gn_ok = a->c_out % 4 == 0 && (p.HW % 64 == 0 || (p.HW >= 8 && p.HW < 64 && 64 % p.HW == 0));
  SSDE_REQUIRE(!a->gn_part || gn_ok, "conv1x1: GroupNorm partials need H*W %% 64 == 0 or a power of two in 8..32");
  p.lHW = ssde_ilog2(p.HW);
  p.gn_entries = p.HW >= 64 ? a->n * (p.HW / 64) : a->n;
  const bool x6 = (a->flags & SSDE_CONVF_BF16X6) != 0;
  {
    const int total = ssde_cdiv(p.m_tiles, 8) * 8 * p.n_tiles;
    const int wgs = (2 * ssde_num_cus() + 7) / 8 * 8;
    const bool pipe_ok = !(a->flags & SSDE_CONVF_NO_GEMM_PIPE) && a->c_out % 4 == 0 && (!a->gn_part || p.HW % 64 == 0) && (!a->chan_add || p.HW % 8 == 0);
    const bool wide_first = a->c_out >= 512 && a->c_out % 256 == 0 && !(a->flags & (SSDE_CONVF_X6_NO_WIDE | SSDE_CONVF_X6_BM64 | SSDE_CONVF_X6_PF2)) &&
                            (long long)ssde_cdiv(p.M, 128) * (a->c_out / 256) >= 2ll * ssde_num_cus();
    const bool pays = x6 && p.K >= 512 && (long long)p.m_tiles * p.n_tiles > wgs && !wide_first;
    if (pipe_ok && x6 && (pays || (a->flags & SSDE_CONVF_GEMM_PIPE))) {
      const int lds = 2 * (x6 ? X6<128>::kStageBytes : kStage * 4) + 4 * kSlabFloats * 4;
      if (lds_out) { *lds_out = lds; return SSDE_OK; }
      const dim3 grid(total < wgs ? total : wgs);
      auto go = [&](auto kfn, std::atomic<bool>& attr_set) {
        if (!attr_set) {
          if (hipFuncSetAttribute(reinterpret_cast<const void*>(kfn), hipFuncAttributeMaxDynamicSharedMemorySize, 160 * 1024) != hipSuccess) return false;
          attr_set = true;
        }
        hipLaunchKernelGGL(kfn, grid, dim3(kThreads), lds, static_cast<hipStream_t>(stream), p);
        return true;
      };
      static std::atomic<bool> pset[2];
      const bool ok = gn ? go(gemm1x1_pipe_kernel<true, true>, pset[0]) : go(gemm1x1_pipe_kernel<false, true>, pset[1]);
      SSDE_REQUIRE(ok, "conv1x1: hipFuncSetAttribute failed");
      SSDE_LAUNCH_CHECK();
      return SSDE_OK;
    }
  }
  int xbm = 128, xpf = 1, xbn = BN;
  if (x6) {
    if (a->flags & SSDE_CONVF_X6_BM64) xbm = 64;
    if (a->flags & SSDE_CONVF_X6_PF2) xpf = 2;
    if ((long long)ssde_cdiv(p.M, 128) * ssde_cdiv(a->c_out, BN) <= ssde_num_cus() && !(a->flags & SSDE_CONVF_X6_WIDE)) xbm = 64;
    const bool wide_fits = a->c_out % 256 == 0 && xbm == 128 && xpf == 1;
    const bool wide_pays = (long long)ssde_cdiv(p.M, 128) * (a->c_out / 256) >= 2ll * ssde_num_cus();
    if (!(a->flags & SSDE_CONVF_X6_NO_WIDE) && wide_fits && (wide_pays || (a->flags & SSDE_CONVF_X6_WIDE))) xbn = 256;
    p.m_tiles = ssde_cdiv(p.M, xbm);
    p.n_tiles = ssde_cdiv(a->c_out, xbn);
  }
  const int lds_ops = x6 ? 2 * (xbn == 256 ? X6<128, 256>::kStageBytes : xbm == 64 ? X6<64>::kStageBytes : X6<128>::kStageBytes) : 2 * kStage * 4;
  const int lds_epi = 64 * (xbn + 4) * 4;
  const int lds = lds_ops > lds_epi ? lds_ops : lds_epi;
  if (lds_out) { *lds_out = lds; return SSDE_OK; }
  const dim3 grid(ssde_cdiv(p.m_tiles, 8) * 8 * p.n_tiles);
  auto go = [&](auto kfn, std::atomic<bool>& attr_set) {
    if (!attr_set) {
      if (hipFuncSetAttribute(reinterpret_cast<const void*>(kfn), hipFuncAttributeMaxDynamicSharedMemorySize, 160 * 1024) != hipSuccess)
        return false;
      attr_set = true;
    }
    hipLaunchKernelGGL(kfn, grid, dim3(kThreads), lds, static_cast<hipStream_t>(stream), p);
    return true;
  };
  static std::atomic<bool> set[12];
  bool ok;
  if (!x6) ok = gn ? go(gemm1x1_kernel<true>, set[0]) : go(gemm1x1_kernel<false>, set[1]);
  else if (xbn == 256) ok = gn ? go(gemm1x1_bf16x6_kernel<true, 128, 1, 256>, set[10]) : go(gemm1x1_bf16x6_kernel<false, 128, 1, 256>, set[11]);
  else if (xbm == 128 && xpf == 1) ok = gn ? go(gemm1x1_bf16x6_kernel<true, 128, 1>, set[2]) : go(gemm1x1_bf16x6_kernel<false, 128, 1>, set[3]);
  else if (xbm == 128) ok = gn ? go(gemm1x1_bf16x6_kernel<true, 128, 2>, set[4]) : go(gemm1x1_bf16x6_kernel<false, 128, 2>, set[5]);
  else if (xpf == 1) ok = gn ? go(gemm1x1_bf16x6_kernel<true, 64, 1>, set[6]) : go(gemm1x1_bf16x6_kernel<false, 64, 1>, set[7]);
  else ok = gn ? go(gemm1x1_bf16x6_kernel<true, 64, 2>, set[8]) : go(gemm1x1_bf16x6_kernel<false, 64, 2>, set[9]);
  SSDE_REQUIRE(ok, "conv1x1: hipFuncSetAttribute failed");
  SSDE_LAUNCH_CHECK();
  return SSDE_OK;
}
```

### score_sde_pytorch_amd/csrc/conv_mfma.hip

```cpp
#include "ssde_common.h"

typedef float f32x16 __attribute__((ext_vector_type(16)));

namespace {

struct ConvGeom {
  int N, Hin, Win, Hout, Wout, Cout, CoutPad;
  int stride, pad;
  int lTW, lTH;
  int tiles_x, tiles_per_img;
  int m_tiles, n_tiles;
};

struct ConvKParams {
  ssde_src main, aux;
  const float* w_main;
  const float* w_aux;
  ConvGeom g;
  const float* bias;
  const float* chan_add;
  int chan_add_ld;
  const float* resid;
  int resid_post;
  float scale;
// ... 441 lines not shown

template <int WM, int WN, int TM, int TN, int BKC3 = 8>
int launch_cfg(ConvPlan& pl, hipStream_t st) {
  dim3 grid(pl.grid), block(kThreads);
  if (pl.kp.ksplit == 2) {
    pl.kp.sync = ssde_conv_sync_slots(pl.kp.g.m_tiles * pl.kp.g.n_tiles);
    SSDE_REQUIRE(pl.kp.sync, "conv: no hand-over slots for a split reduction");
  }
#define SSDE_CONV_LAUNCH(H3, H1)                                                                     \
  do {                                                                                               \
    auto kfn = conv_mfma_kernel<WM, WN, TM, TN, H3, H1, BKC3>;                                       \
    static std::atomic<bool> attr_set{false};             \
    if (!attr_set) {                                                                                 \
      SSDE_HIP_CHECK(hipFuncSetAttribute(reinterpret_cast<const void*>(kfn),                         \
                                         hipFuncAttributeMaxDynamicSharedMemorySize, 160 * 1024));   \
      attr_set = true;                                                                               \
    }                                                                                                \
    hipLaunchKernelGGL(kfn, grid, block, pl.lds_bytes, st, pl.kp);                                   \
  } while (0)
  if (pl.has3 && pl.has1) SSDE_CONV_LAUNCH(true, true);
  else if (pl.has3) SSDE_CONV_LAUNCH(true, false);
  else SSDE_CONV_LAUNCH(false, true);
#undef SSDE_CONV_LAUNCH
  SSDE_LAUNCH_CHECK();
  return SSDE_OK;
}

}

unsigned* ssde_conv_sync_slots(int need) {
  static std::atomic<unsigned> cursor{0};
  if (need <= 0 || need > kSyncSlots / 4) return nullptr;
  unsigned cur = cursor.load(std::memory_order_relaxed), at, next;
  do {
    at = cur % (unsigned)kSyncSlots;
    if (at + (unsigned)need > (unsigned)kSyncSlots) at = 0;
    next = at + (unsigned)need;
  } while (!cursor.compare_exchange_weak(cur, next, std::memory_order_relaxed));
  unsigned* base = nullptr;
  if (hipGetSymbolAddress(reinterpret_cast<void**>(&base), HIP_SYMBOL(g_conv_sync)) != hipSuccess) return nullptr;
  return base + 2 * (size_t)at;
}

typedef int (*ssde_wino_launcher)(const ssde_conv_args*, void*, int*);
static ssde_wino_launcher wino_launcher(int tile) {
  switch (tile) {
    case SSDE_TILE_WINOGRAD: return ssde_conv_wino_launch;
    case SSDE_TILE_WINOGRAD4: return ssde_conv_wino4_launch;
    case SSDE_TILE_WINOGRAD4R: return ssde_conv_wino4r_launch;
    case SSDE_TILE_WINOGRAD4P: return ssde_conv_wino4p_launch;
    default: return nullptr;
  }
}

static int wino_pad_end_ok(const ssde_conv_args* a) {
  SSDE_REQUIRE(!a || a->pad_end == 0 || wino_launcher(a->tile) == nullptr,
               "conv: pad_end %d with Winograd tile %d (end padding runs on the direct kernel only)", a->pad_end, a->tile);
  return SSDE_OK;
}

extern "C" int ssde_conv2d(const ssde_conv_args* a, void* stream) {
  if (int rc = wino_pad_end_ok(a)) return rc;
  if (a && a->gn_in_part0 && !ssde_wino4_xform_merges_gn(a)) {
    const ssde_src& s = a->main;
    SSDE_REQUIRE(s.gn_mean && s.gn_rstd && s.gn_groups > 0 && a->ksize != 0, "conv: gn_in_part0 needs a k x k main source with a GroupNorm prologue");
    ssde_gn_finalize_args f;
    f.part0 = a->gn_in_part0; f.part1 = s.c1 > 0 ? a->gn_in_part1 : nullptr;
    f.c0 = s.c0; f.c1 = s.c1; f.slices0 = a->gn_in_slices0; f.slices1 = s.c1 > 0 ? a->gn_in_slices1 : 0;
    f.n = a->n; f.groups = s.gn_groups; f.eps = a->gn_in_eps;
    f.mean = const_cast<float*>(s.gn_mean); f.rstd = const_cast<float*>(s.gn_rstd);
    if (int rc = ssde_gn_finalize(&f, stream)) return rc;
  }
  if (a) {
    if (ssde_wino_launcher fn = wino_launcher(a->tile)) {
      if (a->tile == SSDE_TILE_WINOGRAD4R && !(a->flags & SSDE_CONVF_V_GIVEN)) {
        int lds = 0;
        if (int rc = fn(a, nullptr, &lds)) return rc;
        if (int rc = ssde_wino4_xform_vq_launch(a, stream)) return rc;
      }
      return fn(a, stream, nullptr);
    }
  }
  if (a && a->dst && ssde_conv1x1_wants(a)) return ssde_conv1x1_launch(a, stream, nullptr);
  if (a && a->dst && ssde_conv_small_wants(a)) return ssde_conv_small_launch(a, stream, nullptr);
  ConvPlan pl;
  if (int rc = make_plan(a, &pl)) return rc;
  hipStream_t st = static_cast<hipStream_t>(stream);
  switch (pl.tile) {
    case SSDE_TILE_256x64: return launch_cfg<4, 1, 2, 2>(pl, st);
    case SSDE_TILE_128x64: return launch_cfg<4, 1, 1, 2>(pl, st);
    case SSDE_TILE_64x64:  return pl.bkc == 8 ? launch_cfg<2, 2, 1, 1>(pl, st) : launch_cfg<2, 2, 1, 1, SSDE_CONV_BKC64>(pl, st);
    case SSDE_TILE_256x32: return launch_cfg<4, 1, 2, 1>(pl, st);
  }
  ssde_set_error("conv: unreachable tile %d", pl.tile);
  return SSDE_EINVAL;
}

extern "C" int ssde_conv_gn_slices(const ssde_conv_args* a) {
  if (!a || a->c_out % 4 != 0) return 0;
  if (wino_pad_end_ok(a)) return 0;
  ssde_conv_args q = *a;
  q.gn_part = nullptr;
  if (ssde_wino_launcher fn = wino_launcher(q.tile)) {
    int s = 0;
    if (fn(&q, reinterpret_cast<void*>(1), &s)) return 0;
    return s;
  }
  if (q.dst && ssde_conv1x1_wants(&q)) {
    const int hw = q.h_out * q.w_out;
    if (hw % 64 == 0) return (hw / 64) * 4;
    return (hw >= 8 && hw < 64 && 64 % hw == 0) ? 4 : 0;
  }
  if (q.dst && ssde_conv_small_wants(&q)) return 0;
  ConvPlan pl;
  if (make_plan(&q, &pl)) return 0;
  return pl.gn_slices;
}

extern "C" int64_t ssde_conv_ws_floats(const ssde_conv_args* a) {
  if (int rc = wino_pad_end_ok(a)) return rc;
  if (a && a->tile == SSDE_TILE_WINOGRAD4P) return ssde_conv_wino4p_ws_floats(a);
  return 0;
}

extern "C" int ssde_conv_lds_bytes(const ssde_conv_args* a) {
  if (int rc = wino_pad_end_ok(a)) return rc;
  if (ssde_wino_launcher fn = a ? wino_launcher(a->tile) : nullptr) {
    int lds = 0;
    if (int rc = fn(a, nullptr, &lds)) return rc;
    return lds;
  }
  if (a && a->dst && ssde_conv1x1_wants(a)) {
    int lds = 0;
    if (int rc = ssde_conv1x1_launch(a, nullptr, &lds)) return rc;
    return lds;
  }
  if (a && a->dst && ssde_conv_small_wants(a)) {
    int lds = 0;
    if (int rc = ssde_conv_small_launch(a, nullptr, &lds)) return rc;
    return lds;
  }
  ConvPlan pl;
  if (int rc = make_plan(a, &pl)) return rc;
  return pl.lds_bytes;
}
```

### score_sde_pytorch_amd/csrc/ssde_common.h

```cpp
#pragma once
#include <hip/hip_runtime.h>
#include <stdint.h>
#include <stdio.h>
#include <stdarg.h>
#include <stdlib.h>
#include <atomic>
#include "../../include/ssde.h"

#define SSDE_OK 0
#define SSDE_EINVAL (-22)
#define SSDE_EHIP (-5)

void ssde_set_error(const char* fmt, ...);
int ssde_conv_wino_launch(const ssde_conv_args* a, void* stream, int* lds_out);
int ssde_conv_wino4_launch(const ssde_conv_args* a, void* stream, int* lds_out);
bool ssde_wino4_xform_merges_gn(const ssde_conv_args* a);
int ssde_wino4_xform_vq_launch(const ssde_conv_args* a, void* stream);
int ssde_conv_wino4r_launch(const ssde_conv_args* a, void* stream, int* lds_out);
int ssde_conv_wino4p_launch(const ssde_conv_args* a, void* stream, int* lds_out);
int64_t ssde_conv_wino4p_ws_floats(const ssde_conv_args* a);
bool ssde_conv1x1_wants(const ssde_conv_args* a);
int ssde_conv1x1_launch(const ssde_conv_args* a, void* stream, int* lds_out);
unsigned* ssde_conv_sync_slots(int need);
int ssde_conv_wino4_splits(int wgs, int ctot, int c_out, unsigned flags);
// ... 310 lines not shown
      for (int b = 0; b < B; ++b)
        if (ok[b]) *reinterpret_cast<float4*>(e.dst + pix[b] * e.Cout + j) = t[b];
      if (stats) {
#pragma unroll
        for (int b = 0; b < B; ++b) {
          if (ok[b]) {
            if (st_n == 0.f) st_p = t[b].x;
            const float d0 = t[b].x - st_p, d1 = t[b].y - st_p, d2 = t[b].z - st_p, d3 = t[b].w - st_p;
            st_s1 += (d0 + d1) + (d2 + d3);
            st_s2 += (d0 * d0 + d1 * d1) + (d2 * d2 + d3 * d3);
            st_n += 4.f;
          }
          if ((((it0 + b + 1) * RSTEP) & rpi_mask) == 0) flush(it0 + b);
        }
      }
#else
#pragma unroll
      for (int b = 0; b < B; ++b) {
        if (ok[b]) {
          float v[4] = {t[b].x + bias4.x + a[b].x, t[b].y + bias4.y + a[b].y, t[b].z + bias4.z + a[b].z, t[b].w + bias4.w + a[b].w};
          const float4 rr = r[b];
          if (!e.resid_post) { v[0] += rr.x; v[1] += rr.y; v[2] += rr.z; v[3] += rr.w; }
#pragma unroll
          for (int k = 0; k < 4; ++k) v[k] *= e.scale;
          if (e.resid_post) { v[0] += rr.x; v[1] += rr.y; v[2] += rr.z; v[3] += rr.w; }
          *reinterpret_cast<float4*>(e.dst + pix[b] * e.Cout + j) = make_float4(v[0], v[1], v[2], v[3]);
          if (stats) {
            if (st_n == 0.f) st_p = v[0];
            const float d0 = v[0] - st_p, d1 = v[1] - st_p, d2 = v[2] - st_p, d3 = v[3] - st_p;
            st_s1 += (d0 + d1) + (d2 + d3);
            st_s2 += (d0 * d0 + d1 * d1) + (d2 * d2 + d3 * d3);
            st_n += 4.f;
          }
        }
        if (stats && (((it0 + b + 1) * RSTEP) & rpi_mask) == 0) flush(it0 + b);
      }
#endif
    }
  } else {
    for (int it = 0; it < ITERS; ++it) {
      const int row = row0 + it * RSTEP;
      size_t pix; int img;
      if (j >= e.Cout || !pixfn(row, pix, img)) continue;
      const float4 t = *reinterpret_cast<const float4*>(tile + row * ld + (SWZ ? (c ^ (((row >> 4) & 1) << 4)) : c));
      const float v[4] = {t.x, t.y, t.z, t.w};
      for (int k = 0; k < 4 && j + k < e.Cout; ++k) {
        float x = v[k];
        if (e.bias) x += e.bias[j + k];
        if (e.chan_add) x += e.chan_add[(size_t)img * e.chan_add_ld + j + k];
        const float r = e.resid ? e.resid[pix * e.Cout + j + k] : 0.f;
        if (e.resid && !e.resid_post) x += r;
        x *= e.scale;
        if (e.resid && e.resid_post) x += r;
        e.dst[pix * e.Cout + j + k] = x;
      }
    }
  }
}


typedef __bf16 ssde_bf16x8 __attribute__((ext_vector_type(8)));
typedef unsigned ssde_u32x4 __attribute__((ext_vector_type(4)));
__device__ __forceinline__ uint32_t ssde_pack_hi16(uint32_t lo, uint32_t hi) {
#ifdef SSDE_EMULATED
  return (hi & 0xffff0000u) | (lo >> 16);
#else
  return __builtin_amdgcn_perm(hi, lo, 0x07060302u);
#endif
}
__device__ __forceinline__ void ssde_split3(const float4& v, uint2& p0, uint2& p1, uint2& p2) {
  const float f[4] = {v.x, v.y, v.z, v.w};
  uint32_t a[4], b[4], c[4];
#pragma unroll
  for (int i = 0; i < 4; ++i) {
    a[i] = __builtin_bit_cast(uint32_t, f[i]);
    const float r = f[i] - __builtin_bit_cast(float, a[i] & 0xffff0000u);
    b[i] = __builtin_bit_cast(uint32_t, r);
    c[i] = __builtin_bit_cast(uint32_t, r - __builtin_bit_cast(float, b[i] & 0xffff0000u));
  }
  p0 = make_uint2(ssde_pack_hi16(a[0], a[1]), ssde_pack_hi16(a[2], a[3]));
  p1 = make_uint2(ssde_pack_hi16(b[0], b[1]), ssde_pack_hi16(b[2], b[3]));
  p2 = make_uint2(ssde_pack_hi16(c[0], c[1]), ssde_pack_hi16(c[2], c[3]));
}
#define SSDE_MFMA_BF16X6(acc, A, B)                                                                                       \
  do {                                                                                                                     \
    acc = __builtin_amdgcn_mfma_f32_32x32x16_bf16(__builtin_bit_cast(ssde_bf16x8, (A)[0]), __builtin_bit_cast(ssde_bf16x8, (B)[2]), acc, 0, 0, 0); \
    acc = __builtin_amdgcn_mfma_f32_32x32x16_bf16(__builtin_bit_cast(ssde_bf16x8, (A)[2]), __builtin_bit_cast(ssde_bf16x8, (B)[0]), acc, 0, 0, 0); \
    acc = __builtin_amdgcn_mfma_f32_32x32x16_bf16(__builtin_bit_cast(ssde_bf16x8, (A)[1]), __builtin_bit_cast(ssde_bf16x8, (B)[1]), acc, 0, 0, 0); \
    acc = __builtin_amdgcn_mfma_f32_32x32x16_bf16(__builtin_bit_cast(ssde_bf16x8, (A)[0]), __builtin_bit_cast(ssde_bf16x8, (B)[1]), acc, 0, 0, 0); \
    acc = __builtin_amdgcn_mfma_f32_32x32x16_bf16(__builtin_bit_cast(ssde_bf16x8, (A)[1]), __builtin_bit_cast(ssde_bf16x8, (B)[0]), acc, 0, 0, 0); \
    acc = __builtin_amdgcn_mfma_f32_32x32x16_bf16(__builtin_bit_cast(ssde_bf16x8, (A)[0]), __builtin_bit_cast(ssde_bf16x8, (B)[0]), acc, 0, 0, 0); \
  } while (0)


__device__ __forceinline__ float ssde_wave_sum(float v) {
#pragma unroll
  for (int o = 32; o > 0; o >>= 1) v += __shfl_xor(v, o, 64);
  return v;
}
__device__ __forceinline__ float ssde_wave_max(float v) {
#pragma unroll
  for (int o = 32; o > 0; o >>= 1) v = fmaxf(v, __shfl_xor(v, o, 64));
  return v;
}
#endif
```

### score_sde_pytorch_amd/engine.py

```python
import ctypes as C
import math
import os

import numpy as np
import torch

from . import _lib as L

_FLT = 4
INV_SQRT2 = float(1.0 / np.sqrt(2.0))

FC_OTHER, FC_CONV3, FC_CONV1, FC_ATTN, FC_GN, FC_FIR = 0, 1, 2, 3, 4, 5

W4P_MIN_BATCH = 16


class Buf:
    __slots__ = ("shape", "numel", "name", "persistent", "tensor", "first", "last")

    def __init__(self, shape, name="", persistent=False):
        self.shape = tuple(int(s) for s in shape)
        self.numel = int(np.prod(self.shape))
        self.name = name
        self.persistent = persistent
# ... 484 lines not shown
    if k.ndim == 1:
        k = np.outer(k, k)
    k = k / np.sum(k)
    return (k * gain).astype(np.float32)


class Lowering:

    def __init__(self, builder, weights, batch):
        self.b, self.w, self.n = builder, weights, batch
        self.parts = {}
        dev = getattr(builder, "device", None)
        self.cus = 256
        if os.environ.get("SSDE_NUM_CUS"):
            self.cus = int(os.environ["SSDE_NUM_CUS"])
        elif dev is not None and torch.device(dev).type == "cuda" and torch.cuda.is_available():
            self.cus = int(torch.cuda.get_device_properties(torch.device(dev)).multi_processor_count)

    def _gn_slices(self, fields):
        if os.environ.get("SSDE_GN_FUSE", "1") == "0":
            return 0
        return int(L.load().ssde_conv_gn_slices(C.byref(self._query_args(fields))))

    def _query_args(self, fields, last=True):
        sub = _expand(L.OP_CONV, fields, 0, 0.0)[-1 if last else 0][0]
        a = L.ConvArgs()
        dummy = 0x1000
        for src_name in ("main", "aux"):
            src, dst = sub[src_name], getattr(a, src_name)
            dst.p0 = dummy if src["p0"] is not None else None
            dst.p1 = dummy if src["p1"] is not None else None
            dst.c0, dst.c1, dst.pro_mode, dst.gn_groups = src["c0"], src["c1"], src["pro_mode"], src["gn_groups"]
            if src["gn_groups"]:
                dst.gn_mean = dst.gn_rstd = dst.gn_gamma = dst.gn_beta = dummy
            if src["drop_thresh"]:
                dst.drop_thresh, dst.drop_seed = src["drop_thresh"], dummy
        a.w_main = dummy if sub["w_main"] is not None else None
        a.w_aux = dummy if sub["w_aux"] is not None else None
        for k in ("n", "h_in", "w_in", "h_out", "w_out", "c_out", "ksize", "stride", "pad", "tile"):
            setattr(a, k, sub[k])
        a.pad_end = sub.get("pad_end", 0)
        a.dst = dummy
        a.flags = sub.get("flags", L.conv_route_flags())
        return a

    def gn_stats(self, t, c, hw, gn_module, t2=None, c2=0):
        ctot = c + c2
        groups = gn_module.num_groups
        mean = self.b.buf(self.n, groups, name="gn_mean")
        rstd = self.b.buf(self.n, groups, name="gn_rstd")
        p0, p1 = self.parts.get(id(t)), (self.parts.get(id(t2)) if t2 is not None else None)
        if p0 is not None and p0[2] == c and (t2 is None or (p1 is not None and p1[2] == c2)) and (ctot // groups) % 4 == 0:
            fin = dict(part0=p0[0], part1=p1[0] if p1 else None, c0=c, c1=c2, slices0=p0[1], slices1=p1[1] if p1 else 0,
                       n=self.n, groups=groups, eps=float(gn_module.eps), mean=mean, rstd=rstd)
            gamma = self.w.vector([gn_module.weight])
            beta = self.w.vector([gn_module.bias])
            assert ctot == gn_module.num_channels
            gn = dict(groups=groups, mean=mean, rstd=rstd, gamma=gamma, beta=beta, pending=fin)
            if os.environ.get("SSDE_GN_MERGE_IN_CONSUMER", "0") != "1":
                self._materialize_stats(gn)
            return gn
        slices = max(1, min(int(math.ceil(256 / self.n)), hw // 64)) if hw >= 128 else 1
        scratch = self.b.buf(self.n * slices * groups * 2, name="gn_scratch") if slices > 1 else None
        self.b.add(L.OP_GN_STATS, dict(p0=t, p1=t2, c0=c, c1=c2, n=self.n, hw=hw, groups=groups, eps=float(gn_module.eps),
                                       mean=mean, rstd=rstd, scratch=scratch, slices=slices), FC_GN)
        gamma = self.w.vector([gn_module.weight])
        beta = self.w.vector([gn_module.bias])
        assert ctot == gn_module.num_channels
        return dict(groups=groups, mean=mean, rstd=rstd, gamma=gamma, beta=beta)

    def _materialize_stats(self, gn, fields=None):
        fin = gn.get("pending") if gn else None
        if fin is None:
            return
        gn["pending"] = None
        if fields is not None:
            fields.update(gn_in_part0=fin["part0"], gn_in_part1=fin["part1"], gn_in_slices0=fin["slices0"],
                          gn_in_slices1=fin["slices1"], gn_in_eps=fin["eps"])
        else:
            self.b.add(L.OP_GN_FINALIZE, fin, FC_GN)

    def conv(self, dst, h_out, w_out, c_out, main=None, w_main=None, h_in=0, w_in=0, stride=1, pad=1,
             aux=None, w_aux=None, bias=None, chan_add=None, chan_add_ld=0, resid=None, scale=1.0, tile=L.TILE_AUTO,
             resid_post=0, wino=False, stats=False, pad_end=0):
        split_tmp = None
        if wino:
            assert main is not None and stride == 1 and pad == 1 and pad_end == 0 and (h_in, w_in) == (h_out, w_out)
            tile = {8: L.TILE_WINOGRAD4P, 6: L.TILE_WINOGRAD4R, 4: L.TILE_WINOGRAD4}.get(wino, L.TILE_WINOGRAD)
            if aux is not None:
                split_tmp = self.b.buf(self.n, h_out, w_out, c_out, name="wino_tmp")
        px = self.n * h_out * w_out
        flops = 0.0
        if main is not None:
            flops += 2.0 * px * 9 * (main["c0"] + main["c1"]) * c_out
        if aux is not None:
            flops += 2.0 * px * (aux["c0"] + aux["c1"]) * c_out
        fields = dict(
            main=main if main is not None else _NOSRC, aux=aux if aux is not None else _NOSRC,
            w_main=w_main, w_aux=w_aux, n=self.n, h_in=h_in, w_in=w_in, h_out=h_out, w_out=w_out, c_out=c_out,
            ksize=3 if main is not None else 0, stride=stride, pad=pad, pad_end=pad_end, tile=tile, bias=bias, chan_add=chan_add,
            chan_add_ld=chan_add_ld, resid_post=resid_post, resid=resid, out_scale=float(scale), dst=dst, gn_part=None,
            wino_v=None, _split_tmp=split_tmp)
        if wino in (4, 6):
            ctot = main["c0"] + main["c1"]
            v_floats = 36 * self.n * (h_out // 4) * (w_out // 4) * ctot
            takes = getattr(self, "emit_wino_v", False) and v_floats * 4 < 2 ** 32 and self._wgrad_takes_wino4(fields)
            if tile == L.TILE_WINOGRAD4R or takes:
                fields["wino_v"] = self.b.buf(v_floats, name="wino_v")
                fields["_v_for_wgrad"] = bool(takes)
        if wino == 8:
            need = int(L.load().ssde_conv_ws_floats(C.byref(self._query_args(fields, last=False))))
            if need <= 0:
                raise L.SsdeError("conv(winograd 4x4, position-batched): %s" % L.load().ssde_last_error().decode())
            fields.update(wino_ws=self.b.buf(need, name="wino_ws"), wino_ws_floats=need)
        if aux is not None:
            self._materialize_stats(aux.get("_gn"))
        if main is not None:
            in_pass = tile == L.TILE_WINOGRAD4R and h_in * w_in >= 64
            self._materialize_stats(main.get("_gn"), fields if in_pass else None)
        if stats and isinstance(dst, Buf):
            slices = self._gn_slices(fields)
            if slices > 0:
                part = self.b.buf(self.n, slices, c_out // 4, 3, name="gn_part")
                fields["gn_part"] = part
                self.parts[id(dst)] = (part, slices, c_out)
        self.b.add(L.OP_CONV, fields, FC_CONV3 if main is not None else FC_CONV1, flops)

    def _wino4_two_kernels(self, h, w, c_out, c_in):
        return os.environ.get("SSDE_WINO4_TWO", "2") != "0" and 36 * self.n * (h // 4) * (w // 4) * c_in * 4 < 2 ** 32 \
            and c_in % 8 == 0

    def _wgrad_takes_wino4(self, f):
        if os.environ.get("SSDE_WINO_V_FROM_FORWARD", "1") == "0":
            return False
        meta = self.w.meta.get(id(f["w_main"]))
        if meta is None or len(meta["parts"]) != 1 or meta["parts"][0]["transpose"]:
            return False
        a = L.WgradArgs()
        s = f["main"]
        a.src.c0, a.src.c1, a.src.pro_mode, a.src.gn_groups = s["c0"], s["c1"], s["pro_mode"], s["gn_groups"]
        a.g_ld, a.g_off = f["c_out"], meta["parts"][0]["row0"]
        a.n, a.h_in, a.w_in, a.h_out, a.w_out = f["n"], f["h_in"], f["w_in"], f["h_out"], f["w_out"]
        a.c_out, a.ksize, a.stride, a.pad = meta["parts"][0]["rows"], 3, f["stride"], f["pad"]
        a.pad_end = f.get("pad_end", 0)
        a.cin_store, a.transpose_out = meta["cin_store"], 0
        a.flags = L.wgrad_route_flags()
        return bool(L.load().ssde_wgrad_wants_winograd4(C.byref(a)))

    def wino_ok(self, h, w, c_out, c_in, aux=False):
        mode = os.environ.get("SSDE_WINOGRAD", "1")
        if mode == "0":
            return 0
        if mode == "1" and h == 4 and w == 4 and not aux and c_in % 32 == 0 and c_out % 64 == 0 and self.n >= W4P_MIN_BATCH:
            return 8
        legal2 = h % 2 == 0 and w % 2 == 0 and h >= 8 and w >= 8 and c_out >= 32 and c_in >= 8 and c_in % 8 == 0
        legal4 = h % 4 == 0 and w % 4 == 0 and h >= 8 and w >= 8 and c_out >= 32 and c_in >= 8 and c_in % 4 == 0
        four = lambda: 6 if self._wino4_two_kernels(h, w, c_out, c_in) else 4
        if mode == "4" and legal4:
            return four()
        if mode == "2" or mode == "4":
            return 2 if legal2 else 0
        n_tiles = -(-c_out // 64)
        if mode != "3" and legal4 and h >= 16 and w >= 16 and -(-(self.n * h * w) // 512) * n_tiles >= self.cus:
            return four()
        if mode != "3" and legal4 and c_in % 16 == 0 and c_in >= 256 and c_out % 4 == 0 \
                and os.environ.get("SSDE_CONV_KSPLIT", "1") != "0":
            wgs4 = -(-(-(-(self.n * h * w) // 512)) // 8) * 8 * n_tiles
            if self.cus // 2 < wgs4 * 2 <= self.cus and self._wino4_two_kernels(h, w, c_out, c_in):
                return 6
            if c_in % 32 == 0 and self.cus // 2 < wgs4 * 4 <= self.cus and self._wino4_two_kernels(h, w, c_out, c_in):
                return 6
        return 2 if legal2 and -(-(self.n * h * w) // 256) * n_tiles >= self.cus // 2 else 0

    def upfirdn(self, src, n_ch, h_in, w_in, taps, up=1, down=1, pad=(0, 0), name="fir"):
        kh, kw = taps.shape
        h_out = (h_in * up + pad[0] + pad[1] - kh) // down + 1
        w_out = (w_in * up + pad[0] + pad[1] - kw) // down + 1
        dst = self.b.buf(self.n, h_out, w_out, n_ch, name=name)
        self._materialize_stats(src.get("_gn"))
        k16 = [0.0] * 16
        for i, v in enumerate(taps.reshape(-1).tolist()):
            k16[i] = float(v)
        self.b.add(L.OP_UPFIRDN, dict(src=src, n=self.n, h_in=h_in, w_in=w_in, c=n_ch, h_out=h_out, w_out=w_out,
                                      up=up, down=down, pad0=pad[0], pad1=pad[1], kh=kh, kw=kw, k=k16, dst=dst), FC_FIR)
        return dst, h_out, w_out
# ... 250 lines not shown
                    hn = b.buf(n, hh, ww, cur_c, name="up_conv")
                    wino = low.wino_ok(hh, ww, cur_c, cur_c)
                    low.conv(hn, hh, ww, cur_c, main=_src(h, cur_c), w_main=self._w3(up.Conv_0, wino=wino), h_in=hh, w_in=ww,
                             bias=self._bias(up.Conv_0), wino=wino, stats=True)
                    h = hn
        assert not hs

        gn_m, conv_m = mods[idx], mods[idx + 1]; idx += 2
        o = self._lower_head(gn_m, conv_m, h, cur_c, hh, ww)
        assert idx == len(mods), (idx, len(mods))
        return o, hh, ww

    def _w3(self, m, cin_pad=None, cout_pad=None, wino=False):
        return self.weights.conv3(m.weight, cin_pad, cout_pad, wino=wino)

    def _w1(self, m, cin_pad=None):
        return self.weights.matrix([(m.weight, False)], cin_pad=cin_pad)

    def _bias(self, m, pad_to=None):
        return self.weights.vector([m.bias], pad_to=pad_to)

    def _shortcut(self, m):
        conv, nin = getattr(m, "Conv_2", None), getattr(m, "NIN_0", None)
        if conv is not None:
            if tuple(conv.weight.shape[2:]) != (1, 1):
                raise NotImplementedError("ResnetBlockDDPM(conv_shortcut=True): the 3x3 shortcut is not lowered (DDPM never sets it)")
            return self._w1(conv), conv.bias
        if nin is not None:
            return self.weights.matrix([(nin.W, True)]), nin.b
        return None, None

    def _res(self, m, t, c, hh, ww, t2=None, c2=0):
        b, low, n = self.b, self.low, self.n
        cin, cout = c + c2, m.out_ch
        assert cin == m.in_ch, (cin, m.in_ch)
        scale = INV_SQRT2 if m.skip_rescale else 1.0
        gn0 = low.gn_stats(t, c, hh * ww, m.GroupNorm_0, t2, c2)
        chan_add, ld = None, 0
        if hasattr(m, "Dense_0") and self._tproj is not None:
            chan_add, ld = (self._tproj, self._tproj_off[id(m.Dense_0)]), self._tproj_ld
        if m.up or m.down:
            assert t2 is None
            if m.up:
                taps = fir_taps(m.fir_kernel, gain=4.0) if m.fir else fir_taps([1, 1], gain=4.0)
                kw = dict(up=2, pad=(2, 1) if m.fir else (1, 0))
            else:
                taps = fir_taps(m.fir_kernel) if m.fir else fir_taps([1, 1])
                kw = dict(down=2, pad=(1, 1) if m.fir else (0, 0))
            hr, ho, wo = low.upfirdn(_src(t, c, pro=L.PRO_GN_SILU, gn=gn0), c, hh, ww, taps, name="res_h_rs", **kw)
            xr, _, _ = low.upfirdn(_src(t, c), c, hh, ww, taps, name="res_x_rs", **kw)
            main0, skip_t, skip_c, skip_t2, skip_c2 = _src(hr, c), xr, c, None, 0
            hh, ww = ho, wo
        else:
            main0 = _src(t, c, t2, c2, pro=L.PRO_GN_SILU, gn=gn0)
            skip_t, skip_c, skip_t2, skip_c2 = t, c, t2, c2
        h1 = b.buf(n, hh, ww, cout, name="res_h1")
        wino0 = low.wino_ok(hh, ww, cout, main0["c0"] + main0["c1"])
        w_short, b_short = self._shortcut(m)
        wino1 = low.wino_ok(hh, ww, cout, cout, aux=w_short is not None)
        low.conv(h1, hh, ww, cout, main=main0, w_main=self._w3(m.Conv_0, wino=wino0), h_in=hh, w_in=ww, bias=self._bias(m.Conv_0),
                 chan_add=chan_add, chan_add_ld=ld, wino=wino0, stats=True)
        gn1 = low.gn_stats(h1, cout, hh * ww, m.GroupNorm_1)
        out = b.buf(n, hh, ww, cout, name="res_out")
        self._n_res += 1
        drop = (float(m.dropout), self.drop_seed, 0x9E3779B1 * self._n_res) if self.drop_seed is not None else None
        main1 = _src(h1, cout, pro=L.PRO_GN_SILU, gn=gn1, drop=drop)
        if w_short is not None:
            bsum = self.weights.vector([m.Conv_1.bias, b_short], mode="sum")
            low.conv(out, hh, ww, cout, main=main1, w_main=self._w3(m.Conv_1, wino=wino1), h_in=hh, w_in=ww,
                     aux=_src(skip_t, skip_c, skip_t2, skip_c2), w_aux=w_short, bias=bsum, scale=scale, wino=wino1,
                     stats=True)
        else:
            assert skip_t2 is None
            low.conv(out, hh, ww, cout, main=main1, w_main=self._w3(m.Conv_1, wino=wino1), h_in=hh, w_in=ww,
                     bias=self._bias(m.Conv_1), resid=skip_t, scale=scale, wino=wino1, stats=True)
        return out, cout

    def _attn(self, m, t, c, hh, ww):
        b, low, n = self.b, self.low, self.n
        gn = low.gn_stats(t, c, hh * ww, m.GroupNorm_0)
        wqkv = self.weights.matrix([(m.NIN_0.W, True), (m.NIN_1.W, True), (m.NIN_2.W, True)])
        bqkv = self.weights.vector([m.NIN_0.b, m.NIN_1.b, m.NIN_2.b])
        qkv = b.buf(n, hh, ww, 3 * c, name="qkv")
        low.conv(qkv, hh, ww, 3 * c, aux=_src(t, c, pro=L.PRO_GN, gn=gn), w_aux=wqkv, bias=bqkv)
        ao = b.buf(n, hh, ww, c, name="attn_o")
        L_ = hh * ww
        b.add(L.OP_ATTN, dict(qkv=qkv, dst=ao, n=n, l=L_, c=c, scale=float(int(c) ** (-0.5))), FC_ATTN,
              4.0 * n * L_ * L_ * c)
        out = b.buf(n, hh, ww, c, name="attn_out")
        low.conv(out, hh, ww, c, aux=_src(ao, c), w_aux=self.weights.matrix([(m.NIN_3.W, True)]),
                 bias=self.weights.vector([m.NIN_3.b]), resid=t,
                 scale=INV_SQRT2 if m.skip_rescale else 1.0, stats=True)
        return out

    def load_inputs(self, x, cond):
        self.x_in.tensor[: x.numel()].copy_(x.reshape(-1))
        self.cond.tensor[: self.n].copy_(cond.reshape(-1).to(torch.float32))
        if self.sig is not self.cond and self.sig.tensor is not None:
            self.sig.tensor[: self.n].copy_(self.model.sigmas.to(torch.float32)[cond.long()])

    def output_view(self):
        return self.out.tensor[: self.n * self.channels * self.h * self.w].view(self.n, self.channels, self.h, self.w)

    def forward(self, x, cond):
        if tuple(x.shape) != (self.n, self.channels, self.h, self.w):
            raise ValueError("engine built for %s, got %s" % ((self.n, self.channels, self.h, self.w), tuple(x.shape)))
        self.weights.refresh()
        self.load_inputs(x.contiguous(), cond)
        self.program.run()
        return self.output_view().clone()

    def flops_per_forward(self):
        return sum(self.program.flops)

    def validate_plans(self):
        lib = L.load()
        out = []
        for i in range(self.program.n):
            op = self.program.ops[i]
            if op.kind == L.OP_CONV:
                r = lib.ssde_conv_lds_bytes(C.byref(op.u.conv))
                if r < 0:
                    raise L.SsdeError("op %d: %s" % (i, lib.ssde_last_error().decode()))
                out.append(r)
        return out
```

### score_sde_pytorch_amd/hipops.py

```python
import ctypes as C

import numpy as np
import torch

from . import _lib as L
from .engine import pack_conv_weight, pack_matrix, pack_wino_weight, pack_wino4_weight, pack_wino4r_weight, pack_wino4p_weight


def _stream():
    return C.c_void_p(torch.cuda.current_stream().cuda_stream)


def _need_cuda(*ts):
    for t in ts:
        if t is not None and not t.is_cuda:
            raise RuntimeError("score_sde_pytorch_amd HIP op called with a %s tensor (no CPU fallback)" % t.device.type)


def _p(t):
    return None if t is None else t.data_ptr()


def _fill_src(s, t, t2=None, pro=L.PRO_NONE, gn=None):
    s.p0, s.c0 = _p(t), t.shape[-1]
    s.p1, s.c1 = (_p(t2), t2.shape[-1]) if t2 is not None else (None, 0)
    s.pro_mode = pro
    if gn is not None:
        mean, rstd, gamma, beta, groups = gn
        s.gn_groups, s.gn_mean, s.gn_rstd, s.gn_gamma, s.gn_beta = groups, _p(mean), _p(rstd), _p(gamma), _p(beta)


def groupnorm_stats(x, groups, eps=1e-6, x2=None, slices=1):
    _need_cuda(x, x2)
    n = x.shape[0]
    hw = int(np.prod(x.shape[1:-1]))
    mean = torch.empty(n, groups, device=x.device)
    rstd = torch.empty(n, groups, device=x.device)
    a = L.GnStatsArgs()
    a.p0, a.c0 = _p(x), x.shape[-1]
    a.p1, a.c1 = (_p(x2), x2.shape[-1]) if x2 is not None else (None, 0)
    a.n, a.hw, a.groups, a.eps = n, hw, groups, eps
    a.mean, a.rstd = _p(mean), _p(rstd)
    scratch = torch.empty(n * slices * groups * 2, device=x.device) if slices > 1 else None
    a.scratch, a.slices = _p(scratch), slices
    L.check(L.load().ssde_groupnorm_stats(C.byref(a), _stream()), "ssde_groupnorm_stats")
    return mean, rstd


def conv2d(x=None, weight=None, bias=None, stride=1, pad=1, x2=None, pro=L.PRO_NONE, gn=None,
           aux=None, aux2=None, aux_weight=None, aux_pro=L.PRO_NONE, aux_gn=None,
           chan_add=None, resid=None, scale=1.0, tile=L.TILE_AUTO, out_hw=None, flags=None, pad_end=0):
    _need_cuda(x, aux, resid)
    a = L.ConvArgs()
    keep = []
    if x is not None:
        n, h_in, w_in = x.shape[0], x.shape[1], x.shape[2]
        c_out = weight.shape[0]
        h_out = (h_in + 2 * pad + pad_end - 3) // stride + 1
        w_out = (w_in + 2 * pad + pad_end - 3) // stride + 1
        if out_hw is not None:
            h_out, w_out = out_hw
        _fill_src(a.main, x, x2, pro, gn)
        packer = {L.TILE_WINOGRAD: pack_wino_weight, L.TILE_WINOGRAD4: pack_wino4_weight,
                  L.TILE_WINOGRAD4R: pack_wino4r_weight, L.TILE_WINOGRAD4P: pack_wino4p_weight}.get(tile, pack_conv_weight)
        wp = packer(weight.to(x.device)); keep.append(wp)
        if tile == L.TILE_WINOGRAD4R:
            wv = torch.empty(36 * n * (h_in // 4) * (w_in // 4) * (x.shape[-1] + (x2.shape[-1] if x2 is not None else 0)), device=x.device)
            keep.append(wv)
            a.wino_v = _p(wv)
        a.w_main, a.ksize, a.stride, a.pad, a.h_in, a.w_in = _p(wp), 3, stride, pad, h_in, w_in
        a.pad_end = pad_end
    else:
        n, h_out, w_out = aux.shape[0], aux.shape[1], aux.shape[2]
        c_out = aux_weight.shape[0]
        a.ksize, a.stride, a.pad = 0, 1, 0
    if aux is not None:
        _fill_src(a.aux, aux, aux2, aux_pro, aux_gn)
        wa = pack_matrix(aux_weight.to(aux.device)); keep.append(wa)
        a.w_aux = _p(wa)
    dev = (x if x is not None else aux).device
    dst = torch.empty(n, h_out, w_out, c_out, device=dev)
    a.n, a.h_out, a.w_out, a.c_out, a.tile = n, h_out, w_out, c_out, tile
    a.bias = _p(bias)
    if chan_add is not None:
        a.chan_add, a.chan_add_ld = _p(chan_add), chan_add.shape[-1]
    a.resid, a.out_scale, a.dst = _p(resid), scale, _p(dst)
    a.flags = L.conv_route_flags() if flags is None else flags
    if tile == L.TILE_WINOGRAD4P:
        need = int(L.load().ssde_conv_ws_floats(C.byref(a)))
        L.check(min(need, 0), "ssde_conv_ws_floats")
        ws = torch.empty(need, device=dev); keep.append(ws)
        a.wino_ws, a.wino_ws_floats = _p(ws), need
    L.check(L.load().ssde_conv2d(C.byref(a), _stream()), "ssde_conv2d")
    return dst


def upfirdn2d_nhwc(x, kernel, up=1, down=1, pad=(0, 0), pro=L.PRO_NONE, gn=None, dual=False, accumulate_into=None):
    _need_cuda(x)
    n, h, w, c = x.shape
    kh, kw = kernel.shape
    h_out = (h * up + pad[0] + pad[1] - kh) // down + 1
    w_out = (w * up + pad[0] + pad[1] - kw) // down + 1
    dst = torch.empty(n, h_out, w_out, c, device=x.device) if accumulate_into is None else accumulate_into
    dst2 = torch.empty(n, h_out, w_out, c, device=x.device) if dual else None
    a = L.UpfirdnArgs()
    _fill_src(a.src, x, None, pro, gn)
    a.accumulate = int(accumulate_into is not None)
    a.dst2 = _p(dst2) if dual else None
    a.n, a.h_in, a.w_in, a.c, a.h_out, a.w_out = n, h, w, c, h_out, w_out
    a.up, a.down, a.pad0, a.pad1, a.kh, a.kw = up, down, pad[0], pad[1], kh, kw
    for i, v in enumerate(np.asarray(kernel.detach().cpu(), dtype=np.float32).reshape(-1).tolist()):
        a.k[i] = v
    a.dst = _p(dst)
    L.check(L.load().ssde_upfirdn2d(C.byref(a), _stream()), "ssde_upfirdn2d")
    return (dst, dst2) if dual else dst


def attention(qkv, channels):
    _need_cuda(qkv)
    n, l = qkv.shape[0], qkv.shape[1]
    dst = torch.empty(n, l, channels, device=qkv.device)
    a = L.AttnArgs()
    a.qkv, a.dst, a.n, a.l, a.c, a.scale = _p(qkv), _p(dst), n, l, channels, float(int(channels) ** (-0.5))
    a.flags = L.attn_route_flags()
    L.check(L.load().ssde_attention(C.byref(a), _stream()), "ssde_attention")
    return dst


def embed(cond, table, dim, kind):
    _need_cuda(cond, table)
    dst = torch.empty(cond.shape[0], dim, device=cond.device)
    a = L.EmbedArgs()
    a.cond, a.w, a.dst, a.n, a.dim, a.kind = _p(cond), _p(table), _p(dst), cond.shape[0], dim, kind
    L.check(L.load().ssde_embed(C.byref(a), _stream()), "ssde_embed")
    return dst


def to_nhwc(x, c_pad=None, a=1.0, b=0.0):
    _need_cuda(x)
    n, c, h, w = x.shape
    c_pad = c_pad or c
    dst = torch.empty(n, h, w, c_pad, device=x.device)
    args = L.ToNhwcArgs()
    args.src, args.dst, args.n, args.c, args.h, args.w, args.c_pad, args.a, args.b = _p(x), _p(dst), n, c, h, w, c_pad, a, b
    L.check(L.load().ssde_to_nhwc(C.byref(args), _stream()), "ssde_to_nhwc")
    return dst


def to_nchw(x, c=None, mode=0, v=None):
    _need_cuda(x)
    n, h, w, c_src = x.shape
    c = c or c_src
    dst = torch.empty(n, c, h, w, device=x.device)
    args = L.ToNchwArgs()
    args.src, args.dst, args.n, args.c, args.h, args.w, args.c_src, args.mode, args.v = _p(x), _p(dst), n, c, h, w, c_src, mode, _p(v)
    L.check(L.load().ssde_to_nchw(C.byref(args), _stream()), "ssde_to_nchw")
    return dst


def fused_bias_act(x, bias=None, channels=1, inner=1, act=1, alpha=0.2, scale=1.0, grad=0, ref=None):
    _need_cuda(x)
    x = x.contiguous()
    dst = torch.empty_like(x)
    a = L.BiasActArgs()
    a.src, a.bias, a.dst, a.numel, a.channels, a.inner, a.act, a.alpha, a.scale = \
        _p(x), _p(bias), _p(dst), x.numel(), channels, inner, act, alpha, scale
    a.grad, a.ref = grad, _p(ref)
    L.check(L.load().ssde_fused_bias_act(C.byref(a), _stream()), "ssde_fused_bias_act")
    return dst


def randn(numel, seed, device, step_ptr=None, stream_id=0):
    dst = torch.empty(numel, device=device)
    a = L.RandnArgs()
    a.dst, a.numel, a.seed, a.step_ptr, a.stream_id = _p(dst), numel, seed, _p(step_ptr), stream_id
    L.check(L.load().ssde_randn(C.byref(a), _stream()), "ssde_randn")
    return dst


def set_dropout(s, p, seed_t, salt):
    s.drop_thresh = min(int(round(p * 2.0 ** 32)), 2 ** 32 - 1) if p > 0 else 0
    s.drop_scale = 1.0 / (1.0 - p) if p > 0 else 1.0
    s.drop_seed = _p(seed_t) if p > 0 else None
    s.drop_salt = salt & 0xFFFFFFFF


def conv_wgrad(x, g, ksize, dw, stride=1, pad=1, x2=None, pro=L.PRO_NONE, gn=None, g_off=0, c_out=None, cin_store=None,
               transpose_out=False, scale=1.0, splits=0, dropout=None, flags=None, pad_end=0):
    _need_cuda(x, g, dw)
    a = L.WgradArgs()
    a.flags = L.wgrad_route_flags() if flags is None else flags
    _fill_src(a.src, x, x2, pro, gn)
    if dropout is not None:
        set_dropout(a.src, *dropout)
    a.g, a.g_ld, a.g_off = _p(g), g.shape[-1], g_off
    a.n, a.h_in, a.w_in, a.h_out, a.w_out = x.shape[0], x.shape[1], x.shape[2], g.shape[1], g.shape[2]
    a.c_out = c_out if c_out is not None else g.shape[-1] - g_off
    ctot = x.shape[-1] + (x2.shape[-1] if x2 is not None else 0)
    a.ksize, a.stride, a.pad, a.pad_end = ksize, stride, pad, pad_end
    a.cin_store = cin_store if cin_store is not None else ctot
    a.transpose_out, a.splits, a.scale, a.dw = int(transpose_out), splits, scale, _p(dw)
    a.splits = 0
    need = wgrad_scratch_floats(a)
    a.splits = splits
    if splits > 1:
        bt = 64 if ksize == 3 else 128
        slab = ksize * ksize * (-(-a.c_out // bt) * bt) * (-(-a.cin_store // bt) * bt)
# ... 172 lines not shown
```

Baseline: 5.563 images/s.

## Emit pre-split bf16 K/V planes from QKV GEMM epilogue for attention

The QKV 1x1 GEMM epilogue now writes K and V directly as 3-way bf16-split planes in the layout the bf16x6 attention producer stages consume. A new attention kernel variant streams these planes with plain 16-byte loads instead of loading fp32 K/V and splitting them itself. This moves the split work out of the attention producer and may shorten its loads, but it adds an extra planes buffer write and turns off the GEMM pipe path for this GEMM. It runs only in inference, with 256 tokens and 128 or 256 channels.

```diff
diff --git a/include/ssde.h b/include/ssde.h
--- a/include/ssde.h
+++ b/include/ssde.h
@@ -8,7 +8,7 @@
 extern "C" {
 #endif
 
-#define SSDE_ABI_VERSION 12
+#define SSDE_ABI_VERSION 13
 
 enum {
   SSDE_PRO_NONE = 0,
@@ -62,6 +62,7 @@
   int32_t pad_end;
   float* wino_ws;
   int64_t wino_ws_floats;
+  void* kv_planes;
 } ssde_conv_args;
 
 enum { SSDE_CONVF_V_GIVEN = 1u,
@@ -76,7 +77,8 @@
        SSDE_CONVF_X6_WIDE = 512u,
        SSDE_CONVF_X6_NO_WIDE = 1024u,
        SSDE_CONVF_KSPLIT2 = 2048u,
-       SSDE_CONVF_KSPLIT4 = 4096u };
+       SSDE_CONVF_KSPLIT4 = 4096u,
+       SSDE_CONVF_KV_PLANES = 8192u };
 enum { SSDE_TILE_AUTO = 0, SSDE_TILE_256x64 = 1, SSDE_TILE_128x64 = 2, SSDE_TILE_64x64 = 3, SSDE_TILE_256x32 = 4,
        SSDE_TILE_WINOGRAD = 5,
        SSDE_TILE_WINOGRAD4 = 6,
@@ -116,8 +118,10 @@
   int32_t n, l, c; float scale;
   uint32_t flags;
   int32_t _pad0;
+  const void* kv_planes;
 } ssde_attn_args;
-enum { SSDE_ATTNF_BF16X6 = 1u };
+enum { SSDE_ATTNF_BF16X6 = 1u,
+       SSDE_ATTNF_KV_PLANES = 2u };
 
 typedef struct ssde_embed_args {
   const float* cond;
diff --git a/score_sde_pytorch_amd/_lib.py b/score_sde_pytorch_amd/_lib.py
--- a/score_sde_pytorch_amd/_lib.py
+++ b/score_sde_pytorch_amd/_lib.py
@@ -3,7 +3,7 @@
 
 _HERE = os.path.dirname(os.path.abspath(__file__))
 LIB_PATH = os.environ.get("SSDE_LIB_PATH") or os.path.join(_HERE, "libssde_hip.so")
-ABI_VERSION = 12
+ABI_VERSION = 13
 
 PRO_NONE, PRO_GN, PRO_GN_SILU, PRO_SILU = 0, 1, 2, 3
 TILE_AUTO, TILE_256x64, TILE_128x64, TILE_64x64, TILE_256x32, TILE_WINOGRAD, TILE_WINOGRAD4 = 0, 1, 2, 3, 4, 5, 6
@@ -11,7 +11,8 @@
 TILE_WINOGRAD4P = 10
 TILES_WINOGRAD4 = (TILE_WINOGRAD4, TILE_WINOGRAD4R, TILE_WINOGRAD4P)
 CONVF_V_GIVEN, CONVF_BF16X6, CONVF_NO_KSPLIT, CONVF_BKC8, CONVF_GEMM_PIPE, CONVF_NO_GEMM_PIPE, CONVF_X6_BM64, CONVF_X6_PF2, \
-    CONVF_NO_SMALL_COUT, CONVF_X6_WIDE, CONVF_X6_NO_WIDE, CONVF_KSPLIT2, CONVF_KSPLIT4 = 1, 2, 4, 8, 16, 32, 64, 128, 256, 512, 1024, 2048, 4096
+    CONVF_NO_SMALL_COUT, CONVF_X6_WIDE, CONVF_X6_NO_WIDE, CONVF_KSPLIT2, CONVF_KSPLIT4, CONVF_KV_PLANES = \
+    1, 2, 4, 8, 16, 32, 64, 128, 256, 512, 1024, 2048, 4096, 8192
 WGRADF_DIRECT, WGRADF_F2, WGRADF_F4_FORCE, WGRADF_NO_STREAMK, WGRADF_NO_XCD_ORDER, WGRADF_1X1_CHUNKED, WGRADF_XVEC1 = 1, 2, 4, 8, 16, 32, 64
 GNBWDF_THREE_KERNELS, GNBWDF_DEFER_PARAMS = 1, 2
 (OP_CONV, OP_GN_STATS, OP_UPFIRDN, OP_ATTN, OP_EMBED, OP_TO_NHWC, OP_TO_NCHW, OP_BIAS_ACT, OP_SUMSQ,
@@ -41,7 +42,7 @@
                 ("bias", _fp), ("chan_add", _fp), ("chan_add_ld", C.c_int32), ("resid_post", C.c_int32),
                 ("resid", _fp), ("out_scale", C.c_float), ("flags", C.c_uint32), ("dst", _fp), ("gn_part", _fp), ("wino_v", _fp),
                 ("gn_in_part0", _fp), ("gn_in_part1", _fp), ("gn_in_slices0", C.c_int32), ("gn_in_slices1", C.c_int32),
-                ("gn_in_eps", C.c_float), ("pad_end", C.c_int32), ("wino_ws", _fp), ("wino_ws_floats", C.c_int64)]
+                ("gn_in_eps", C.c_float), ("pad_end", C.c_int32), ("wino_ws", _fp), ("wino_ws_floats", C.c_int64), ("kv_planes", _fp)]
 
 
 class GnStatsArgs(C.Structure):
@@ -88,7 +89,7 @@
 
 class AttnArgs(C.Structure):
     _fields_ = [("qkv", _fp), ("dst", _fp), ("n", C.c_int32), ("l", C.c_int32), ("c", C.c_int32), ("scale", C.c_float),
-                ("flags", C.c_uint32), ("_pad0", C.c_int32)]
+                ("flags", C.c_uint32), ("_pad0", C.c_int32), ("kv_planes", _fp)]
 
 
 class EmbedArgs(C.Structure):
@@ -302,12 +303,17 @@
     return f
 
 
-ATTNF_BF16X6 = 1
+ATTNF_BF16X6, ATTNF_KV_PLANES = 1, 2
 
 
 def attn_route_flags(env=None):
     e = os.environ if env is None else env
     return ATTNF_BF16X6 if e.get("SSDE_MATRIX", "").startswith("b") and e.get("SSDE_ATTN_X6", "1") != "0" else 0
+
+
+def kv_planes_wanted(env=None):
+    e = os.environ if env is None else env
+    return e.get("SSDE_ATTN_KV_PLANES", "1") != "0"
 
 
 def wgrad_route_flags(env=None):
diff --git a/score_sde_pytorch_amd/backward.py b/score_sde_pytorch_amd/backward.py
--- a/score_sde_pytorch_amd/backward.py
+++ b/score_sde_pytorch_amd/backward.py
@@ -107,6 +107,7 @@
 
 
 class TrainEngine(E.UNetEngine):
+    lowers_backward = True
 
     def __init__(self, model, batch, height, width, device, vp_score=False, input_grad=False, dropout=True,
                  param_grads=True):
diff --git a/score_sde_pytorch_amd/csrc/attention.hip b/score_sde_pytorch_amd/csrc/attention.hip
--- a/score_sde_pytorch_amd/csrc/attention.hip
+++ b/score_sde_pytorch_amd/csrc/attention.hip
@@ -1,5 +1,6 @@
 #include "ssde_common.h"
 #include <type_traits>
+#include <utility>
 
 typedef float f32x16 __attribute__((ext_vector_type(16)));
 
@@ -231,10 +232,18 @@
   b = __builtin_bit_cast(uint32_t, r);
   c = __builtin_bit_cast(uint32_t, r - __builtin_bit_cast(float, b & 0xffff0000u));
 }
-}
-
-template <int kNst>
-__global__ __launch_bounds__(x6::kT) void attn_x6_kernel(const float* __restrict__ qkv, float* __restrict__ dst, int N, float scale) {
+constexpr int loads_behind(int e, int last, int nst, int nk, int nv) {
+  int c = 0;
+  for (int x = e + 1; x <= last; ++x) c += x < nst ? nk : nv;
+  return c;
+}
+template <class F, int... I>
+__device__ __forceinline__ void static_for(F&& f, std::integer_sequence<int, I...>) { (f(std::integral_constant<int, I>{}), ...); }
+}
+
+template <int kNst, bool kPlanes>
+__device__ __forceinline__ void attn_x6_body(const float* __restrict__ qkv, float* __restrict__ dst, int N, float scale,
+                                             const char* __restrict__ planes) {
   using namespace x6;
   constexpr int C = 16 * kNst;
   SSDE_LDS(smem);
@@ -358,9 +367,50 @@
     }
   };
 
-  ssde_f32x4 R[4][4];
-  zero();
-  if (!consumer) { request(0, R[0]); request(1, R[1]); request(2, R[2]); request(3, R[3]); }
+  constexpr int kNK = 6, kNV = C * 6 / 256;
+  static_assert(!kPlanes || C == 128 || C == 256, "a V stage is a whole number of 4 KB rounds of the producer half");
+  const char* pimg = planes + (kPlanes ? (size_t)n * 12 * kL * C : 0);
+  const uint32_t poff = (uint32_t)ptid * 16u;
+  auto request_p = [&](auto E, auto& Rs) __attribute__((always_inline)) {
+    constexpr int e = decltype(E)::value;
+    constexpr int nld = e < nst ? kNK : kNV;
+    const char* sb = pimg + (e < nst ? e * kKStage : nst * kKStage + (e - nst) * (3 * C * 32));
+#pragma unroll
+    for (int i = 0; i < nld; i += 2) {
+      const char* sbi = sb + (i + 1) * 4096;
+      SSDE_GLOAD16_I_SAFE(Rs[i], poff, sbi, -4096);
+      if (i + 1 < nld) SSDE_GLOAD16_I_SAFE(Rs[i + 1], poff, sbi, 0);
+    }
+  };
+  auto park_p = [&](auto E, const auto& Rs, char* buf) __attribute__((always_inline)) {
+    constexpr int e = decltype(E)::value;
+    constexpr int nld = e < nst ? kNK : kNV;
+#pragma unroll
+    for (int i = 0; i < nld; ++i) *reinterpret_cast<ssde_f32x4*>(buf + i * 4096 + poff) = Rs[i];
+  };
+#define behind(e, last) x6::loads_behind((e), (last), nst, kNK, kNV)
+#ifdef SSDE_EMULATED
+#define SSDE_X6P_WAIT(E, n, Rs) ((void)0)
+#else
+#define SSDE_X6P_WAIT(E, n, Rs)                                                                                                   \
+  do {                                                                                                                            \
+    if constexpr ((E) < nst || kNV == 6)                                                                                          \
+      asm volatile("s_waitcnt vmcnt(%6)" : "+v"((Rs)[0]), "+v"((Rs)[1]), "+v"((Rs)[2]), "+v"((Rs)[3]), "+v"((Rs)[4]), "+v"((Rs)[5]) : "n"(n) : "memory"); \
+    else                                                                                                                          \
+      asm volatile("s_waitcnt vmcnt(%3)" : "+v"((Rs)[0]), "+v"((Rs)[1]), "+v"((Rs)[2]) : "n"(n) : "memory");                      \
+  } while (0)
+#endif
+  using I0 = std::integral_constant<int, 0>;
+
+  ssde_f32x4 R[4][kPlanes ? 6 : 4];
+  if constexpr (!kPlanes) zero();
+  if (!consumer) {
+    if constexpr (kPlanes) {
+      x6::static_for([&](auto E) __attribute__((always_inline)) { request_p(E, R[decltype(E)::value]); }, std::make_integer_sequence<int, 2>{});
+    } else {
+      request(0, R[0]); request(1, R[1]); request(2, R[2]); request(3, R[3]);
+    }
+  }
   {
     const int cq4 = C >> 2, total = kRows * cq4;
     for (int item0 = tid; item0 < total; item0 += 8 * kT) {
@@ -387,6 +437,7 @@
     }
   }
   if (consumer) {
+    if constexpr (kPlanes) zero();
     SSDE_LDS_BARRIER();
     for (int u = 0; u < nst; ++u) {
       Frags f;
@@ -394,6 +445,22 @@
       mfmas(Eight{}, f);
       SSDE_LDS_BARRIER();
     }
+  } else if constexpr (kPlanes) {
+    request_p(std::integral_constant<int, 2>{}, R[2]);
+    request_p(std::integral_constant<int, 3>{}, R[3]);
+    SSDE_X6P_WAIT(0, behind(0, 3), R[0]);
+    park_p(I0{}, R[0], stage0);
+    SSDE_LDS_BARRIER();
+    x6::static_for([&](auto U) __attribute__((always_inline)) {
+      constexpr int u = decltype(U)::value, j = u & 3, jn = (j + 1) & 3;
+      request_p(std::integral_constant<int, u + 4>{}, R[j]);
+      SSDE_X6P_WAIT(u + 1, behind(u + 1, u + 4), R[jn]);
+      if constexpr (u + 1 < nst) park_p(std::integral_constant<int, u + 1>{}, R[jn], (j & 1) ? stage0 : stage1);
+      SSDE_LDS_BARRIER();
+    }, std::make_integer_sequence<int, nst>{});
+    SSDE_X6P_WAIT(nst + 1, behind(nst + 1, nst + 3), R[1]);
+    SSDE_X6P_WAIT(nst + 2, behind(nst + 2, nst + 3), R[2]);
+    SSDE_X6P_WAIT(nst + 3, 0, R[3]);
   } else {
     SSDE_X6_WAIT(12, R[0]);
     park_k(R[0], stage0);
@@ -481,6 +548,18 @@
           }
       }
     }
+  } else if constexpr (kPlanes) {
+    park_p(std::integral_constant<int, nst>{}, R[0], stage0);
+    SSDE_LDS_BARRIER();
+    x6::static_for([&](auto V) __attribute__((always_inline)) {
+      constexpr int v = decltype(V)::value, j = v & 3, jn = (j + 1) & 3;
+      if constexpr (v + 4 < 16) request_p(std::integral_constant<int, nst + v + 4>{}, R[j]);
+      if constexpr (v + 1 < 16) {
+        if constexpr (v + 1 >= 4) SSDE_X6P_WAIT(nst + v + 1, behind(nst + v + 1, nst + (v + 4 < 16 ? v + 4 : 15)), R[jn]);
+        park_p(std::integral_constant<int, nst + v + 1>{}, R[jn], (j & 1) ? stage0 : stage1);
+      }
+      SSDE_LDS_BARRIER();
+    }, std::make_integer_sequence<int, 16>{});
   } else {
     park_v(R[0], stage0);
     SSDE_LDS_BARRIER();
@@ -501,6 +580,18 @@
     }
   }
 #undef SSDE_X6_WAIT
+#undef SSDE_X6P_WAIT
+#undef behind
+}
+
+template <int kNst>
+__global__ __launch_bounds__(x6::kT) void attn_x6_kernel(const float* __restrict__ qkv, float* __restrict__ dst, int N, float scale) {
+  attn_x6_body<kNst, false>(qkv, dst, N, scale, nullptr);
+}
+template <int kNst>
+__global__ __launch_bounds__(x6::kT) void attn_x6p_kernel(const float* __restrict__ qkv, float* __restrict__ dst, int N, float scale,
+                                                          const char* __restrict__ planes) {
+  attn_x6_body<kNst, true>(qkv, dst, N, scale, planes);
 }
 
 __global__ __launch_bounds__(256) void attn_bwd_q_kernel(const float* __restrict__ qkv, const float* __restrict__ o,
@@ -639,8 +730,12 @@
   SSDE_REQUIRE(a && a->qkv && a->dst, "attention: null args");
   SSDE_REQUIRE(a->n > 0 && a->l > 0 && a->l <= kLMax, "attention: token count %d outside 1..%d", a->l, kLMax);
   SSDE_REQUIRE(a->c > 0 && a->c % 32 == 0, "attention: channels must be a multiple of 32 (got %d)", a->c);
+  const bool kv_planes = (a->flags & SSDE_ATTNF_KV_PLANES) != 0;
+  SSDE_REQUIRE(!kv_planes || ((a->flags & SSDE_ATTNF_BF16X6) && a->kv_planes && a->l == x6::kL && (a->c == 128 || a->c == 256)),
+               "attention: SSDE_ATTNF_KV_PLANES needs SSDE_ATTNF_BF16X6, kv_planes, 256 tokens and 128 or 256 channels (got l %d, c %d)", a->l, a->c);
   if ((a->flags & SSDE_ATTNF_BF16X6) && a->l == x6::kL && a->c <= 256 && a->c % 64 == 0) {
-    static std::atomic<bool> x6_set[4];
+    static std::atomic<bool> x6_set[6];
+    const char* planes = static_cast<const char*>(a->kv_planes);
     const dim3 grid(ssde_cdiv(a->n, 8) * 8 * 4);
     hipStream_t st = static_cast<hipStream_t>(stream);
 #define SSDE_ATTN_X6_GO(NST, SLOT)                                                                       \
@@ -648,6 +743,14 @@
       if (int rc = set_lds_once(attn_x6_kernel<NST>, x6::kLds, &x6_set[SLOT])) return rc;                \
       hipLaunchKernelGGL(attn_x6_kernel<NST>, grid, dim3(x6::kT), x6::kLds, st, a->qkv, a->dst, a->n, a->scale); \
     } while (0)
+#define SSDE_ATTN_X6P_GO(NST, SLOT)                                                                      \
+    do {                                                                                                 \
+      if (int rc = set_lds_once(attn_x6p_kernel<NST>, x6::kLds, &x6_set[SLOT])) return rc;               \
+      hipLaunchKernelGGL(attn_x6p_kernel<NST>, grid, dim3(x6::kT), x6::kLds, st, a->qkv, a->dst, a->n, a->scale, planes); \
+    } while (0)
+    if (kv_planes) {
+      if (a->c == 128) SSDE_ATTN_X6P_GO(8, 4); else SSDE_ATTN_X6P_GO(16, 5);
+    } else
     switch (a->c) {
       case 64: SSDE_ATTN_X6_GO(4, 0); break;
       case 128: SSDE_ATTN_X6_GO(8, 1); break;
@@ -655,6 +758,7 @@
       default: SSDE_ATTN_X6_GO(16, 3); break;
     }
 #undef SSDE_ATTN_X6_GO
+#undef SSDE_ATTN_X6P_GO
     SSDE_LAUNCH_CHECK();
     return SSDE_OK;
   }
diff --git a/score_sde_pytorch_amd/csrc/conv1x1.hip b/score_sde_pytorch_amd/csrc/conv1x1.hip
--- a/score_sde_pytorch_amd/csrc/conv1x1.hip
+++ b/score_sde_pytorch_amd/csrc/conv1x1.hip
@@ -50,6 +50,8 @@
   float* dst;
   float* gn_part;
   int lHW, gn_entries;
+  char* kv_planes;
+  int kv_c;
 };
 
 template <bool kGn>
@@ -237,7 +239,7 @@
   static constexpr int NBW = kBN / 64;
 };
 
-template <bool kGn, int kBM, int kPF, int kBN = 128>
+template <bool kGn, int kBM, int kPF, int kBN = 128, bool kKv = false>
 __global__ __launch_bounds__(kThreads, kBN == 256 ? 2 : (kBM == 64 ? 4 : 3) - (kPF == 2 ? SSDE_X6_PF2_OCC_LOSS : 0)) void gemm1x1_bf16x6_kernel(const GemmParams p) {
   using X = X6<kBM, kBN>;
   constexpr int NA = X::NA, NB = X::NBW, NBW = X::NBW, RS = 64;
@@ -447,6 +449,11 @@
           }
     }
     __syncthreads();
+    if (kKv && n0 >= p.kv_c) {
+      const int mh = m0 + half * 64;
+      const bool is_v = n0 >= 2 * p.kv_c;
+      ssde_store_kv_planes<kBN, kThreads>(smem, LDT, e, n0, is_v, p.kv_c, n0 - (is_v ? 2 : 1) * p.kv_c, mh >> 8, mh & 255, p.kv_planes);
+    } else
     ssde_store_tile<64, kBN, kThreads, SSDE_GEMM_BATCH>(smem, LDT, n0, e, [&](int row, size_t& pix, int& img) {
       const int m = m0 + half * 64 + row;
       if (m >= p.M) return false;
@@ -785,10 +792,21 @@
   p.lHW = ssde_ilog2(p.HW);
   p.gn_entries = p.HW >= 64 ? a->n * (p.HW / 64) : a->n;
   const bool x6 = (a->flags & SSDE_CONVF_BF16X6) != 0;
+  const bool kv = (a->flags & SSDE_CONVF_KV_PLANES) != 0;
+  p.kv_planes = nullptr; p.kv_c = 0;
+  if (kv) {
+    SSDE_REQUIRE(x6, "conv1x1: SSDE_CONVF_KV_PLANES needs SSDE_CONVF_BF16X6");
+    SSDE_REQUIRE(a->kv_planes != nullptr, "conv1x1: SSDE_CONVF_KV_PLANES without kv_planes");
+    SSDE_REQUIRE(p.HW == 256 && a->c_out % 3 == 0 && (a->c_out / 3) % 128 == 0 && a->c_out / 3 <= 256,
+                 "conv1x1: kv planes need 256 tokens per image and c_out = 3 C, C = 128 or 256 (got %d tokens, c_out %d)", p.HW, a->c_out);
+    SSDE_REQUIRE(!a->resid && !a->gn_part, "conv1x1: kv planes with a residual or GroupNorm partials");
+    SSDE_REQUIRE(!(a->flags & SSDE_CONVF_X6_PF2), "conv1x1: kv planes with SSDE_CONVF_X6_PF2 (no such instantiation)");
+    p.kv_planes = static_cast<char*>(a->kv_planes); p.kv_c = a->c_out / 3;
+  }
   {
     const int total = ssde_cdiv(p.m_tiles, 8) * 8 * p.n_tiles;
     const int wgs = (2 * ssde_num_cus() + 7) / 8 * 8;
-    const bool pipe_ok = !(a->flags & SSDE_CONVF_NO_GEMM_PIPE) && a->c_out % 4 == 0 && (!a->gn_part || p.HW % 64 == 0) && (!a->chan_add || p.HW % 8 == 0);
+    const bool pipe_ok = !kv && !(a->flags & SSDE_CONVF_NO_GEMM_PIPE) && a->c_out % 4 == 0 && (!a->gn_part || p.HW % 64 == 0) && (!a->chan_add || p.HW % 8 == 0);
     const bool wide_first = a->c_out >= 512 && a->c_out % 256 == 0 && !(a->flags & (SSDE_CONVF_X6_NO_WIDE | SSDE_CONVF_X6_BM64 | SSDE_CONVF_X6_PF2)) &&
                             (long long)ssde_cdiv(p.M, 128) * (a->c_out / 256) >= 2ll * ssde_num_cus();
     const bool pays = x6 && p.K >= 512 && (long long)p.m_tiles * p.n_tiles > wgs && !wide_first;
@@ -816,7 +834,7 @@
     if (a->flags & SSDE_CONVF_X6_BM64) xbm = 64;
     if (a->flags & SSDE_CONVF_X6_PF2) xpf = 2;
     if ((long long)ssde_cdiv(p.M, 128) * ssde_cdiv(a->c_out, BN) <= ssde_num_cus() && !(a->flags & SSDE_CONVF_X6_WIDE)) xbm = 64;
-    const bool wide_fits = a->c_out % 256 == 0 && xbm == 128 && xpf == 1;
+    const bool wide_fits = a->c_out % 256 == 0 && xbm == 128 && xpf == 1 && (!kv || p.kv_c % 256 == 0);
     const bool wide_pays = (long long)ssde_cdiv(p.M, 128) * (a->c_out / 256) >= 2ll * ssde_num_cus();
     if (!(a->flags & SSDE_CONVF_X6_NO_WIDE) && wide_fits && (wide_pays || (a->flags & SSDE_CONVF_X6_WIDE))) xbn = 256;
     p.m_tiles = ssde_cdiv(p.M, xbm);
@@ -836,9 +854,12 @@
     hipLaunchKernelGGL(kfn, grid, dim3(kThreads), lds, static_cast<hipStream_t>(stream), p);
     return true;
   };
-  static std::atomic<bool> set[12];
+  static std::atomic<bool> set[18];
   bool ok;
-  if (!x6) ok = gn ? go(gemm1x1_kernel<true>, set[0]) : go(gemm1x1_kernel<false>, set[1]);
+  if (kv && xbn == 256) ok = gn ? go(gemm1x1_bf16x6_kernel<true, 128, 1, 256, true>, set[12]) : go(gemm1x1_bf16x6_kernel<false, 128, 1, 256, true>, set[13]);
+  else if (kv && xbm == 128) ok = gn ? go(gemm1x1_bf16x6_kernel<true, 128, 1, 128, true>, set[14]) : go(gemm1x1_bf16x6_kernel<false, 128, 1, 128, true>, set[15]);
+  else if (kv) ok = gn ? go(gemm1x1_bf16x6_kernel<true, 64, 1, 128, true>, set[16]) : go(gemm1x1_bf16x6_kernel<false, 64, 1, 128, true>, set[17]);
+  else if (!x6) ok = gn ? go(gemm1x1_kernel<true>, set[0]) : go(gemm1x1_kernel<false>, set[1]);
   else if (xbn == 256) ok = gn ? go(gemm1x1_bf16x6_kernel<true, 128, 1, 256>, set[10]) : go(gemm1x1_bf16x6_kernel<false, 128, 1, 256>, set[11]);
   else if (xbm == 128 && xpf == 1) ok = gn ? go(gemm1x1_bf16x6_kernel<true, 128, 1>, set[2]) : go(gemm1x1_bf16x6_kernel<false, 128, 1>, set[3]);
   else if (xbm == 128) ok = gn ? go(gemm1x1_bf16x6_kernel<true, 128, 2>, set[4]) : go(gemm1x1_bf16x6_kernel<false, 128, 2>, set[5]);
diff --git a/score_sde_pytorch_amd/csrc/conv_mfma.hip b/score_sde_pytorch_amd/csrc/conv_mfma.hip
--- a/score_sde_pytorch_amd/csrc/conv_mfma.hip
+++ b/score_sde_pytorch_amd/csrc/conv_mfma.hip
@@ -547,6 +547,7 @@
     }
   }
   if (a && a->dst && ssde_conv1x1_wants(a)) return ssde_conv1x1_launch(a, stream, nullptr);
+  SSDE_REQUIRE(!a || !(a->flags & SSDE_CONVF_KV_PLANES), "conv2d: SSDE_CONVF_KV_PLANES on a launch the bf16x6 GEMM does not take");
   if (a && a->dst && ssde_conv_small_wants(a)) return ssde_conv_small_launch(a, stream, nullptr);
   ConvPlan pl;
   if (int rc = make_plan(a, &pl)) return rc;
diff --git a/score_sde_pytorch_amd/csrc/ssde_common.h b/score_sde_pytorch_amd/csrc/ssde_common.h
--- a/score_sde_pytorch_amd/csrc/ssde_common.h
+++ b/score_sde_pytorch_amd/csrc/ssde_common.h
@@ -416,6 +416,60 @@
   p1 = make_uint2(ssde_pack_hi16(b[0], b[1]), ssde_pack_hi16(b[2], b[3]));
   p2 = make_uint2(ssde_pack_hi16(c[0], c[1]), ssde_pack_hi16(c[2], c[3]));
 }
+template <int NCOLS, int NT>
+__device__ __forceinline__ void ssde_store_kv_planes(const float* tile, int ld, const SsdeEpi& e, int j0, bool is_v, int C, int ch0,
+                                                     int img, int tok0, char* planes) {
+  auto value = [&](float t, float bias, float add) {
+    float v = t + bias + add;
+    if (!e.resid_post) v += 0.f;
+    v *= e.scale;
+    if (e.resid_post) v += 0.f;
+    return v;
+  };
+  char* base = planes + (size_t)img * 12 * 256 * C;
+  const float* ca = e.chan_add ? e.chan_add + (size_t)img * e.chan_add_ld + j0 : nullptr;
+  const float4 z4 = make_float4(0.f, 0.f, 0.f, 0.f);
+  if (!is_v) {
+    for (int i = threadIdx.x; i < 64 * (NCOLS / 16); i += NT) {
+      const int key = i & 63, c = (i >> 6) * 16;
+      uint2 q[3][4];
+#pragma unroll
+      for (int k = 0; k < 4; ++k) {
+        const float4 t = *reinterpret_cast<const float4*>(tile + key * ld + c + 4 * k);
+        const float4 b = e.bias ? *reinterpret_cast<const float4*>(e.bias + j0 + c + 4 * k) : z4;
+        const float4 a = ca ? *reinterpret_cast<const float4*>(ca + c + 4 * k) : z4;
+        ssde_split3(make_float4(value(t.x, b.x, a.x), value(t.y, b.y, a.y), value(t.z, b.z, a.z), value(t.w, b.w, a.w)),
+                    q[0][k], q[1][k], q[2][k]);
+      }
+      char* d = base + (size_t)((ch0 + c) >> 4) * (3 * 256 * 32) + (tok0 + key) * 32;
+#pragma unroll
+      for (int p = 0; p < 3; ++p) {
+        *reinterpret_cast<uint4*>(d + p * (256 * 32)) = make_uint4(q[p][0].x, q[p][0].y, q[p][1].x, q[p][1].y);
+        *reinterpret_cast<uint4*>(d + p * (256 * 32) + 16) = make_uint4(q[p][2].x, q[p][2].y, q[p][3].x, q[p][3].y);
+      }
+    }
+  } else {
+    for (int i = threadIdx.x; i < NCOLS * 4; i += NT) {
+      const int ch = i % NCOLS, tg = i / NCOLS;
+      const float b = e.bias ? e.bias[j0 + ch] : 0.f;
+      const float a = ca ? ca[ch] : 0.f;
+      uint2 q[3][4];
+#pragma unroll
+      for (int k = 0; k < 4; ++k) {
+        const float* t = tile + (tg * 16 + 4 * k) * ld + ch;
+        ssde_split3(make_float4(value(t[0], b, a), value(t[ld], b, a), value(t[2 * ld], b, a), value(t[3 * ld], b, a)),
+                    q[0][k], q[1][k], q[2][k]);
+      }
+      char* d = base + (size_t)(C >> 4) * (3 * 256 * 32) + (size_t)((tok0 >> 4) + tg) * (3 * C * 32) + (ch0 + ch) * 32;
+#pragma unroll
+      for (int p = 0; p < 3; ++p) {
+        *reinterpret_cast<uint4*>(d + p * (C * 32)) = make_uint4(q[p][0].x, q[p][0].y, q[p][1].x, q[p][1].y);
+        *reinterpret_cast<uint4*>(d + p * (C * 32) + 16) = make_uint4(q[p][2].x, q[p][2].y, q[p][3].x, q[p][3].y);
+      }
+    }
+  }
+}
+
 #define SSDE_MFMA_BF16X6(acc, A, B)                                                                                       \
   do {                                                                                                                     \
     acc = __builtin_amdgcn_mfma_f32_32x32x16_bf16(__builtin_bit_cast(ssde_bf16x8, (A)[0]), __builtin_bit_cast(ssde_bf16x8, (B)[2]), acc, 0, 0, 0); \
diff --git a/score_sde_pytorch_amd/engine.py b/score_sde_pytorch_amd/engine.py
--- a/score_sde_pytorch_amd/engine.py
+++ b/score_sde_pytorch_amd/engine.py
@@ -590,7 +590,7 @@
 
     def conv(self, dst, h_out, w_out, c_out, main=None, w_main=None, h_in=0, w_in=0, stride=1, pad=1,
              aux=None, w_aux=None, bias=None, chan_add=None, chan_add_ld=0, resid=None, scale=1.0, tile=L.TILE_AUTO,
-             resid_post=0, wino=False, stats=False, pad_end=0):
+             resid_post=0, wino=False, stats=False, pad_end=0, kv_planes=None, flags=None):
         split_tmp = None
         if wino:
             assert main is not None and stride == 1 and pad == 1 and pad_end == 0 and (h_in, w_in) == (h_out, w_out)
@@ -609,6 +609,8 @@
             ksize=3 if main is not None else 0, stride=stride, pad=pad, pad_end=pad_end, tile=tile, bias=bias, chan_add=chan_add,
             chan_add_ld=chan_add_ld, resid_post=resid_post, resid=resid, out_scale=float(scale), dst=dst, gn_part=None,
             wino_v=None, _split_tmp=split_tmp)
+        if kv_planes is not None:
+            fields.update(kv_planes=kv_planes, flags=flags)
         if wino in (4, 6):
             ctot = main["c0"] + main["c1"]
             v_floats = 36 * self.n * (h_out // 4) * (w_out // 4) * ctot
@@ -1025,11 +1027,19 @@
         wqkv = self.weights.matrix([(m.NIN_0.W, True), (m.NIN_1.W, True), (m.NIN_2.W, True)])
         bqkv = self.weights.vector([m.NIN_0.b, m.NIN_1.b, m.NIN_2.b])
         qkv = b.buf(n, hh, ww, 3 * c, name="qkv")
-        low.conv(qkv, hh, ww, 3 * c, aux=_src(t, c, pro=L.PRO_GN, gn=gn), w_aux=wqkv, bias=bqkv)
+        L_ = hh * ww
+        conv_flags, attn_flags = L.conv_route_flags(), L.attn_route_flags()
+        planes = None
+        if (L_ == 256 and c in (128, 256) and not self.train and not self.input_grad and not getattr(self, "lowers_backward", False)
+                and (conv_flags & L.CONVF_BF16X6) and (attn_flags & L.ATTNF_BF16X6) and L.kv_planes_wanted()):
+            planes = b.buf(n, L_, 3 * c, name="kv_planes")
+        low.conv(qkv, hh, ww, 3 * c, aux=_src(t, c, pro=L.PRO_GN, gn=gn), w_aux=wqkv, bias=bqkv,
+                 kv_planes=planes, flags=(conv_flags | L.CONVF_KV_PLANES) if planes is not None else None)
         ao = b.buf(n, hh, ww, c, name="attn_o")
-        L_ = hh * ww
-        b.add(L.OP_ATTN, dict(qkv=qkv, dst=ao, n=n, l=L_, c=c, scale=float(int(c) ** (-0.5))), FC_ATTN,
-              4.0 * n * L_ * L_ * c)
+        attn = dict(qkv=qkv, dst=ao, n=n, l=L_, c=c, scale=float(int(c) ** (-0.5)))
+        if planes is not None:
+            attn.update(kv_planes=planes, flags=attn_flags | L.ATTNF_KV_PLANES)
+        b.add(L.OP_ATTN, attn, FC_ATTN, 4.0 * n * L_ * L_ * c)
         out = b.buf(n, hh, ww, c, name="attn_out")
         low.conv(out, hh, ww, c, aux=_src(ao, c), w_aux=self.weights.matrix([(m.NIN_3.W, True)]),
                  bias=self.weights.vector([m.NIN_3.b]), resid=t,
diff --git a/score_sde_pytorch_amd/hipops.py b/score_sde_pytorch_amd/hipops.py
--- a/score_sde_pytorch_amd/hipops.py
+++ b/score_sde_pytorch_amd/hipops.py
@@ -49,7 +49,7 @@
 
 def conv2d(x=None, weight=None, bias=None, stride=1, pad=1, x2=None, pro=L.PRO_NONE, gn=None,
            aux=None, aux2=None, aux_weight=None, aux_pro=L.PRO_NONE, aux_gn=None,
-           chan_add=None, resid=None, scale=1.0, tile=L.TILE_AUTO, out_hw=None, flags=None, pad_end=0):
+           chan_add=None, resid=None, scale=1.0, tile=L.TILE_AUTO, out_hw=None, flags=None, pad_end=0, kv_planes=False):
     _need_cuda(x, aux, resid)
     a = L.ConvArgs()
     keep = []
@@ -86,13 +86,18 @@
         a.chan_add, a.chan_add_ld = _p(chan_add), chan_add.shape[-1]
     a.resid, a.out_scale, a.dst = _p(resid), scale, _p(dst)
     a.flags = L.conv_route_flags() if flags is None else flags
+    planes = None
+    if kv_planes:
+        dst.zero_()
+        planes = torch.zeros(n, 6 * h_out * w_out * (c_out // 3), dtype=torch.int16, device=dev)
+        a.kv_planes, a.flags = _p(planes), a.flags | L.CONVF_KV_PLANES
     if tile == L.TILE_WINOGRAD4P:
         need = int(L.load().ssde_conv_ws_floats(C.byref(a)))
         L.check(min(need, 0), "ssde_conv_ws_floats")
         ws = torch.empty(need, device=dev); keep.append(ws)
         a.wino_ws, a.wino_ws_floats = _p(ws), need
     L.check(L.load().ssde_conv2d(C.byref(a), _stream()), "ssde_conv2d")
-    return dst
+    return (dst, planes) if kv_planes else dst
 
 
 def upfirdn2d_nhwc(x, kernel, up=1, down=1, pad=(0, 0), pro=L.PRO_NONE, gn=None, dual=False, accumulate_into=None):
@@ -116,13 +121,16 @@
     return (dst, dst2) if dual else dst
 
 
-def attention(qkv, channels):
+def attention(qkv, channels, kv_planes=None):
     _need_cuda(qkv)
     n, l = qkv.shape[0], qkv.shape[1]
     dst = torch.empty(n, l, channels, device=qkv.device)
     a = L.AttnArgs()
     a.qkv, a.dst, a.n, a.l, a.c, a.scale = _p(qkv), _p(dst), n, l, channels, float(int(channels) ** (-0.5))
     a.flags = L.attn_route_flags()
+    if kv_planes is not None:
+        _need_cuda(kv_planes)
+        a.kv_planes, a.flags = _p(kv_planes), a.flags | L.ATTNF_KV_PLANES
     L.check(L.load().ssde_attention(C.byref(a), _stream()), "ssde_attention")
     return dst
 
```

New measurement: 5.472 images/s. -1.6%, worse.
